# ZencashOfficial/ginger-lib

Measured on AMD Instinct MI355X. Metric: MNT4-753 G1 MSM scalar-muls/sec + 2^n NTT ms at 1/2/4/8 MI355X, higher is better.
Workload: dtype u32 (29-bit limbs of 753-bit Montgomery residues, 64-bit accumulators)

## Files before the change

ginger-lib_amd/__init__.py:

```python
import ctypes
import os

import numpy as np

_PKG_DIR = os.path.dirname(os.path.abspath(__file__))
LIB_PATH = os.path.join(_PKG_DIR, "libginger_hip.so")

GH_OK = 0
FFT_INVERSE = 1
FFT_COSET = 2

CURVES = {"mnt4753_g1": 0, "mnt4753_g2": 1, "mnt6753_g1": 2, "mnt6753_g2": 3}
CURVE_DEG = {"mnt4753_g1": 1, "mnt4753_g2": 2, "mnt6753_g1": 1, "mnt6753_g2": 3}
FIELDS = {"mnt4753_fr": 0, "mnt6753_fr": 1}

ABI_SYMBOLS = [
    "gh_init", "gh_shutdown", "gh_last_error", "gh_device_name",
    "gh_msm", "gh_bases_upload", "gh_bases_upload_wire", "gh_bases_generate_chain", "gh_bases_download", "gh_bases_free", "gh_bases_len", "gh_bases_precompute", "gh_bases_precomputed_window", "gh_bases_precompute_rows", "gh_bases_table_rows",
    "gh_msm_resident", "gh_msm_resident_dev", "gh_msm_resident_dev_batch",
    "gh_msm_cached", "gh_key_cache_config", "gh_key_cache_clear", "gh_key_cache_stats", "gh_bases_content_hash",
    "gh_bases_key_id", "gh_test_hooks",
    "gh_msm_set_window", "gh_msm_set_affine", "gh_msm_set_dedup", "gh_msm_get_window", "gh_msm_last_timing", "gh_msm_batch_timing",
    "gh_domain_supported", "gh_fft", "gh_fft_dev", "gh_vec_mul_dev", "gh_vec_sub_dev", "gh_vec_scale_dev",
    "gh_vec_mul", "gh_vec_scale", "gh_fft_last_kernel_ms", "gh_measure_fpmul_peak", "gh_kernel_resources", "gh_witness_map", "gh_witness_map_dev",
# ... 159 lines not shown

    def download(self, dtype=np.uint64):
        out = np.empty(self.nbytes // np.dtype(dtype).itemsize, dtype=dtype)
        _check(load_library().gh_dev_download(_ptr(out), self.ptr, out.nbytes))
        return out

    def free(self):
        if self.ptr:
            load_library().gh_dev_free(self.ptr)
            self.ptr = ctypes.c_void_p()

    def __enter__(self):
        return self

    def __exit__(self, *exc):
        self.free()


def msm_cached(curve, bases, scalars, infinity=None):
    deg = CURVE_DEG[curve]
    bases = _u64(bases, 24 * deg)
    scalars = _u64(scalars, 12)
    inf = None if infinity is None else np.ascontiguousarray(infinity, dtype=np.uint8)
    out = np.zeros(36 * deg, dtype=np.uint64)
    _check(load_library().gh_msm_cached(CURVES[curve], _ptr(bases), _ptr(inf) if inf is not None else None, bases.size // (24 * deg),
                                        _ptr(scalars), scalars.size // 12, _ptr(out)))
    return out


def key_cache_config(max_bytes=None, table_after=2):
    _check(load_library().gh_key_cache_config((1 << 64) - 1 if max_bytes is None else int(max_bytes), int(table_after)))


def key_cache_clear():
    _check(load_library().gh_key_cache_clear())


def key_cache_stats():
    st = KeyCacheStats()
    _check(load_library().gh_key_cache_stats(ctypes.byref(st)))
    return {k: int(getattr(st, k)) for k, _ in KeyCacheStats._fields_}


def bases_content_hash(curve, bases, infinity=None):
    deg = CURVE_DEG[curve]
    bases = _u64(bases, 24 * deg)
    inf = None if infinity is None else np.ascontiguousarray(infinity, dtype=np.uint8)
    hi = ctypes.c_uint64(0)
    lo = load_library().gh_bases_content_hash(CURVES[curve], _ptr(bases), _ptr(inf) if inf is not None else None, bases.size // (24 * deg), ctypes.byref(hi))
    return int(lo), int(hi.value)


def measure_fpmul_peak():
    v = ctypes.c_double(0)
    _check(load_library().gh_measure_fpmul_peak(ctypes.byref(v)))
    return float(v.value)


def kernel_resources(which):
    a, b, c = ctypes.c_uint32(0), ctypes.c_uint32(0), ctypes.c_uint32(0)
    _check(load_library().gh_kernel_resources(which.encode(), ctypes.byref(a), ctypes.byref(b), ctypes.byref(c)))
    return {"scratch_bytes_per_lane": int(a.value), "registers": int(b.value), "lds_bytes": int(c.value)}


def acc_stamps(max_records=1 << 16):
    buf = np.zeros((max_records, 16), dtype=np.uint32)
    n = ctypes.c_uint32(0)
    fn = load_library().gh_acc_stamps_read
    fn.argtypes = [ctypes.POINTER(ctypes.c_uint32), ctypes.c_size_t, ctypes.POINTER(ctypes.c_uint32)]
    _check(fn(buf.ctypes.data_as(ctypes.POINTER(ctypes.c_uint32)), buf.size, ctypes.byref(n)))
    return buf[:int(n.value)]


def bases_key_id(curve, bases, infinity=None):
    deg = CURVE_DEG[curve]
    bases = _u64(bases, 24 * deg)
    inf = None if infinity is None else np.ascontiguousarray(infinity, dtype=np.uint8)
    out = (ctypes.c_uint64 * 4)()
    _check(load_library().gh_bases_key_id(CURVES[curve], _ptr(bases), _ptr(inf) if inf is not None else None, bases.size // (24 * deg), out))
    return tuple(int(x) for x in out)


def set_test_hooks(flags):
    _check(load_library().gh_test_hooks(int(flags)))


class ResidentBases:

    def __init__(self, curve, bases, infinity=None):
        self.curve = curve
        deg = CURVE_DEG[curve]
        bases = _u64(bases, 24 * deg)
        n = bases.size // (24 * deg)
        inf = None
        if infinity is not None:
            inf = np.ascontiguousarray(infinity, dtype=np.uint8)
            assert inf.size == n
        self.handle = ctypes.c_void_p()
        _check(load_library().gh_bases_upload(CURVES[curve], _ptr(bases), _ptr(inf) if inf is not None else None, n,
                                               ctypes.byref(self.handle)))
        self.n = n

    @classmethod
    def from_wire(cls, curve, data):
        buf = np.frombuffer(bytes(data), dtype=np.uint8)
        rec = 192 * CURVE_DEG[curve] + 1
        if buf.size % rec:
            raise ValueError("wire data is not a multiple of %d bytes" % rec)
        self = cls.__new__(cls)
        self.curve = curve
        self.n = buf.size // rec
        self.handle = ctypes.c_void_p()
        _check(load_library().gh_bases_upload_wire(CURVES[curve], _ptr(buf), self.n, ctypes.byref(self.handle)))
        return self

    @classmethod
    def chain(cls, curve, p0_xy, step_xy, n):
        self = cls.__new__(cls)
        self.curve, self.n = curve, int(n)
        self.handle = ctypes.c_void_p()
        p0, st = _u64(p0_xy), _u64(step_xy)
        _check(load_library().gh_bases_generate_chain(CURVES[curve], _ptr(p0), _ptr(st), self.n, ctypes.byref(self.handle)))
        return self

    def download(self, first, count):
        out = np.zeros((int(count), 24 * CURVE_DEG[self.curve]), dtype=np.uint64)
        _check(load_library().gh_bases_download(self.handle, int(first), int(count), _ptr(out)))
        return out

    def precompute(self, window_bits=0, max_rows=0):
        _check(load_library().gh_bases_precompute_rows(self.handle, int(window_bits), int(max_rows)))
        return load_library().gh_bases_precomputed_window(self.handle)

    def table_rows(self):
        return load_library().gh_bases_table_rows(self.handle)

    def msm(self, scalars):
        scalars = _u64(scalars, 12)
        out = np.zeros(36 * CURVE_DEG[self.curve], dtype=np.uint64)
        _check(load_library().gh_msm_resident(self.handle, _ptr(scalars), scalars.size // 12, _ptr(out)))
        return out

    def msm_dev(self, d_scalars, n_scalars):
        out = np.zeros(36 * CURVE_DEG[self.curve], dtype=np.uint64)
        _check(load_library().gh_msm_resident_dev(self.handle, d_scalars.ptr, n_scalars, _ptr(out)))
        return out

    def free(self):
        if self.handle:
            load_library().gh_bases_free(self.handle)
            self.handle = ctypes.c_void_p()


def msm_batch_dev(jobs):
    if not jobs:
        return []
    k = len(jobs)
    deg = CURVE_DEG[jobs[0][0].curve]
    handles = (ctypes.c_void_p * k)(*[j[0].handle for j in jobs])
    scal = (ctypes.c_void_p * k)(*[j[1].ptr for j in jobs])
    ns = (ctypes.c_size_t * k)(*[int(j[2]) for j in jobs])
    out = np.zeros(k * 36 * deg, dtype=np.uint64)
    _check(load_library().gh_msm_resident_dev_batch(handles, scal, ns, k, _ptr(out)))
    return [out[i * 36 * deg:(i + 1) * 36 * deg].copy() for i in range(k)]


class VariableBaseMSM:

    @staticmethod
    def multi_scalar_mul(curve, bases, scalars, infinity=None):
        deg = CURVE_DEG[curve]
        bases = _u64(bases, 24 * deg)
        scalars = _u64(scalars, 12)
        n_b, n_s = bases.size // (24 * deg), scalars.size // 12
        inf = None
        if infinity is not None:
            inf = np.ascontiguousarray(infinity, dtype=np.uint8)
            assert inf.size == n_b
        out = np.zeros(36 * deg, dtype=np.uint64)
        _check(load_library().gh_msm(CURVES[curve], _ptr(bases), _ptr(inf) if inf is not None else None, n_b,
                                      _ptr(scalars), n_s, _ptr(out)))
        return out


class FixedBaseMSM:

    @staticmethod
    def get_mul_window_size(num_scalars):
        return load_library().gh_fixed_base_window(int(num_scalars))

    def __init__(self, curve, g_xyz, scalar_size=753, window=None, num_scalars=0):
        self.curve = curve
        self.window = int(window) if window else self.get_mul_window_size(num_scalars)
        g = _u64(g_xyz)
        assert g.size == 36 * CURVE_DEG[curve]
        self.handle = ctypes.c_void_p()
        _check(load_library().gh_fixed_base_table(CURVES[curve], _ptr(g), int(scalar_size), self.window, ctypes.byref(self.handle)))

    def multi_scalar_mul(self, scalars):
        s = _u64(scalars, 12)
        n = s.size // 12
        out = np.zeros((n, 36 * CURVE_DEG[self.curve]), dtype=np.uint64)
        _check(load_library().gh_fixed_base_msm(self.handle, _ptr(s), n, _ptr(out)))
        return out

    def multi_scalar_mul_affine(self, scalars, canonical=False):
        s = _u64(scalars, 12)
        n = s.size // 12
        xy = np.zeros((n, 24 * CURVE_DEG[self.curve]), dtype=np.uint64)
        inf = np.zeros(n, dtype=np.uint8)
        _check(load_library().gh_fixed_base_msm_affine(self.handle, _ptr(s), n, _ptr(xy), _ptr(inf), 1 if canonical else 0))
        return xy, inf

    def free(self):
        if self.handle:
            load_library().gh_fixed_base_free(self.handle)
            self.handle = ctypes.c_void_p()


def msm_set_window(c):
    _check(load_library().gh_msm_set_window(int(c)))


def msm_set_affine(mode):
    _check(load_library().gh_msm_set_affine(int(mode)))


def msm_set_dedup(on):
    _check(load_library().gh_msm_set_dedup(1 if on else 0))


def dev_trim():
    _check(load_library().gh_dev_trim())


def msm_last_timing():
    t = MsmTiming()
    _check(load_library().gh_msm_last_timing(ctypes.byref(t)))
    return {k: getattr(t, k) for k, _ in MsmTiming._fields_}


def msm_batch_timing(index):
    t = MsmTiming()
    _check(load_library().gh_msm_batch_timing(int(index), ctypes.byref(t)))
    return {k: getattr(t, k) for k, _ in MsmTiming._fields_}


def proj_add(curve, acc, p):
    acc = _u64(acc).copy()
    p = _u64(p)
    _check(load_library().gh_proj_add(CURVES[curve], _ptr(acc), _ptr(p)))
    return acc


def proj_mul(curve, xyz, scalar12):
    xyz = _u64(xyz)
    k = _u64(scalar12, 12)
    out = np.zeros_like(xyz)
    _check(load_library().gh_proj_mul(CURVES[curve], _ptr(xyz), _ptr(k), _ptr(out)))
    return out


def proj_neg(curve, xyz):
    out = _u64(xyz).copy()
    _check(load_library().gh_proj_neg(CURVES[curve], _ptr(out)))
    return out


_FIELD_ONE = {}


def field_one(curve):
    if curve not in _FIELD_ONE:
        deg = CURVE_DEG[curve]
        z = proj_mul(curve, np.zeros(36 * deg, dtype=np.uint64), np.zeros(12, dtype=np.uint64))
        _FIELD_ONE[curve] = z[12 * deg:24 * deg].copy()
    return _FIELD_ONE[curve]


def proj_to_affine(curve, xyz):
    deg = CURVE_DEG[curve]
    xyz = _u64(xyz)
    out = np.zeros(24 * deg, dtype=np.uint64)
    inf = np.zeros(1, dtype=np.uint8)
    _check(load_library().gh_proj_to_affine(CURVES[curve], _ptr(xyz), _ptr(out), _ptr(inf)))
    return out, bool(inf[0])


class EvaluationDomain:

    def __init__(self, field, num_coeffs):
        lg = ctypes.c_uint32()
        ok = load_library().gh_domain_supported(FIELDS[field], int(num_coeffs), ctypes.byref(lg))
        if not ok:
            raise GingerHipError("domain of 2^%d exceeds the 2-adicity of %s" % (lg.value, field))
        self.field = field
        self.log_size_of_group = lg.value
        self.size = 1 << lg.value

    @classmethod
    def new(cls, field, num_coeffs):
        try:
            return cls(field, num_coeffs)
        except GingerHipError:
            return None

    def _run(self, a, flags):
        a = _u64(a, 12)
        out = np.empty(self.size * 12, dtype=np.uint64)
        _check(load_library().gh_fft(FIELDS[self.field], _ptr(a), a.size // 12, _ptr(out), self.log_size_of_group, flags))
        return out

    def fft(self, coeffs):
        return self._run(coeffs, 0)

    def ifft(self, evals):
        return self._run(evals, FFT_INVERSE)
# ... 64 lines not shown
```

ginger-lib_amd/csrc/ginger_hip.hip:

```cpp
#include <atomic>
#include <condition_variable>
#include <exception>
#include <new>
#include <random>
#include <thread>
#include <stdlib.h>
#include <string.h>
#include <vector>
#include "runtime.h"
#include "scan_kernels.h"
#include "asm_kernels.h"

namespace gh_rt {

Ctx g;
std::string g_err;
static std::mutex g_mu;
std::mutex& api_mutex() { return g_mu; }
static char g_devname[256] = "";
static int g_device_req = -1;

int ensure_init() {
    if (g.ready) return GH_OK;
    int count = 0;
    hipError_t e = hipGetDeviceCount(&count);
    if (e != hipSuccess || count == 0) {
        g_err = "no HIP device visible (this library has no CPU fallback)";
        return GH_E_NO_DEVICE;
    }
    int dev = 0;
    const char* lr = getenv("LOCAL_RANK");
    if (g_device_req >= 0) dev = g_device_req;
    else if (lr) dev = atoi(lr) % count;
    g.device = dev;
    HIPCHK(hipSetDevice(dev));
    hipDeviceProp_t prop;
    HIPCHK(hipGetDeviceProperties(&prop, dev));
    g.num_cus = prop.multiProcessorCount > 0 ? prop.multiProcessorCount : 256;
    snprintf(g_devname, sizeof g_devname, "%s, %d CUs, %s", prop.name, prop.multiProcessorCount, prop.gcnArchName);
    if (strncmp(prop.gcnArchName, "gfx950", 6) != 0) {
        g_err = std::string("device is not gfx950: ") + prop.gcnArchName;
        return GH_E_NO_DEVICE;
    }
    HIPCHK(hipStreamCreate(&g.stream));
    {
        int least = 0, greatest = 0;
        HIPCHK(hipDeviceGetStreamPriorityRange(&least, &greatest));
        auto prio = [&](const char* env, int dflt) {
            const char* v = getenv(env);
            if (!v) return dflt;
            if (!strcmp(v, "low")) return least;
            if (!strcmp(v, "high")) return greatest;
            return (least + greatest) / 2;
        };
        HIPCHK(hipStreamCreateWithPriority(&g.stream_acc, hipStreamDefault, prio("GH_PRIO_ACC", least)));
        HIPCHK(hipStreamCreateWithPriority(&g.stream_red, hipStreamDefault, prio("GH_PRIO_RED", greatest)));
        HIPCHK(hipStreamCreateWithPriority(&g.stream_acc2, hipStreamDefault, prio("GH_PRIO_ACC", least)));
        if (msm_knobs().acc_alt) HIPCHK(hipStreamCreateWithPriority(&g.stream_acc_alt, hipStreamDefault, prio("GH_PRIO_ACC", least)));
    }
    for (auto& ev : g.tev) HIPCHK(hipEventCreateWithFlags(&ev, hipEventDisableTiming));
    for (auto& ev : g.ev) HIPCHK(hipEventCreate(&ev));
    for (auto& sl : g.pev) for (auto& ev : sl) HIPCHK(hipEventCreate(&ev));
    g.ready = true;
    return GH_OK;
}

int api_exception() noexcept {
    int rc = GH_E_HIP;
    const char* what = "unknown C++ exception";
    char buf[384];
    try {
        throw;
    } catch (const std::bad_alloc&) {
        rc = GH_E_NOMEM;
        what = "out of host memory (std::bad_alloc)";
    } catch (const std::exception& e) {
        snprintf(buf, sizeof buf, "C++ exception inside the library: %s", e.what());
        what = buf;
    } catch (...) {
    }
    try {
        std::lock_guard<std::mutex> lk(g_mu);
        g_err = what;
    } catch (...) {
    }
    return rc;
}

int scratch_guard(const void* kernel, size_t threads) {
    static std::map<const void*, size_t> frames;
    size_t& reserved = g.scratch_reserved;
    auto it = frames.find(kernel);
    if (it == frames.end()) {
        hipFuncAttributes a;
        memset(&a, 0, sizeof a);
        size_t f = 0;
        if (hipFuncGetAttributes(&a, kernel) == hipSuccess) f = a.localSizeBytes;
        else (void)hipGetLastError();
        it = frames.emplace(kernel, f).first;
    }
    const size_t frame = it->second;
    if (frame < 1024) return GH_OK;
    const size_t resident = (size_t)g.num_cus * 32 * 64;
    const size_t lanes = threads < resident ? (threads + 63) / 64 * 64 : resident;
    const size_t need = frame * lanes;
    if (need <= reserved) return GH_OK;
    size_t free_b = 0, total_b = 0;
    if (hipMemGetInfo(&free_b, &total_b) != hipSuccess) { (void)hipGetLastError(); return GH_OK; }
    const size_t margin = (size_t)256 << 20;
    if (free_b < need - reserved + margin) {
        char b[256];
        snprintf(b, sizeof b, "not enough device memory for the kernel's stack frames: %zu B per lane x %zu lanes = %zu MB of scratch, %zu MB free",
                 frame, lanes, need >> 20, free_b >> 20);
        g_err = b;
        return GH_E_NOMEM;
    }
    reserved = need;
    return GH_OK;
}

int pool_get(const char* name, size_t bytes, void** out) {
    DevBuf& b = g.pool[name];
    if (b.cap < bytes) {
        if (b.p) {
            HIPCHK(hipDeviceSynchronize());
            HIPCHK(hipFree(b.p));
            b.p = nullptr;
            b.cap = 0;
        }
        size_t cap = bytes + bytes / 8 + 256;
        HIPCHK(hipMalloc(&b.p, cap));
        b.cap = cap;
    }
    *out = b.p;
    return GH_OK;
}

size_t pool_cap(const char* name) {
    auto it = g.pool.find(name);
    return it == g.pool.end() ? 0 : it->second.cap;
}
void pool_release(const char* prefix) {
    const size_t len = strlen(prefix);
    for (auto it = g.pool.begin(); it != g.pool.end();) {
        if (it->first.compare(0, len, prefix) == 0) {
            if (it->second.p) (void)hipFree(it->second.p);
            it = g.pool.erase(it);
        } else {
            ++it;
        }
    }
}
void pool_trim(const char* prefix, size_t keep_bytes) {
    const size_t len = strlen(prefix);
    bool synced = false;
    for (auto it = g.pool.begin(); it != g.pool.end();) {
        if (it->first.compare(0, len, prefix) != 0 || it->second.cap <= keep_bytes) {
            ++it;
            continue;
        }
        if (!synced) (void)hipStreamSynchronize(g.stream);
        synced = true;
        (void)hipFree(it->second.p);
        it = g.pool.erase(it);
    }
}

int device_scan(const uint32_t* in, uint32_t* out, size_t n, const char* tmpname, hipStream_t stream) {
    using namespace gh;
    if (!stream) stream = g.stream;
    size_t per_block = (size_t)SCAN_BLOCK * SCAN_ITEMS;
    size_t nblocks = (n + per_block - 1) / per_block;
    uint32_t* sums;
    int rc = pool_get(tmpname, (nblocks + 1) * 4, (void**)&sums);
    if (rc) return rc;
    GH_LAUNCH(scan_partials_kernel, dim3((unsigned)nblocks), dim3(SCAN_BLOCK), 0, stream, in, sums, n);
    GH_LAUNCH(scan_block_sums_kernel, dim3(1), dim3(1024), 0, stream, sums, nblocks);
    GH_LAUNCH(scan_final_kernel, dim3((unsigned)nblocks), dim3(SCAN_BLOCK), 0, stream, in, sums, out, n);
    HIPCHK(hipGetLastError());
    return GH_OK;
}

const MsmOps* ops_of(gh_curve_t curve) {
    switch (curve) {
        case GH_MNT4753_G1: return msm_ops_mnt4753_g1();
        case GH_MNT4753_G2: return msm_ops_mnt4753_g2();
        case GH_MNT6753_G1: return msm_ops_mnt6753_g1();
        case GH_MNT6753_G2: return msm_ops_mnt6753_g2();
        default: g_err = "unknown curve id"; return nullptr;
    }
}

static int to_device(void* d_dst, const void* h_src, size_t bytes) {
    HIPCHK(hipMemcpyAsync(d_dst, h_src, bytes, hipMemcpyHostToDevice, g.stream));
    return GH_OK;
}
static int to_host_sync(void* h_dst, const void* d_src, size_t bytes) {
    HIPCHK(hipMemcpyAsync(h_dst, d_src, bytes, hipMemcpyDeviceToHost, g.stream));
    HIPCHK(hipStreamSynchronize(g.stream));
    return GH_OK;
}

}

using namespace gh_rt;

extern "C" {

int gh_init(const int* devices, int n_devices) try {
    std::lock_guard<std::mutex> lk(g_mu);
    if (g.ready) return GH_OK;
    if (devices && n_devices > 0) {
        int count = 0;
        if (hipGetDeviceCount(&count) != hipSuccess || count == 0) { g_err = "no HIP device visible"; return GH_E_NO_DEVICE; }
        if (devices[0] < 0 || devices[0] >= count) { g_err = "device index out of range"; return GH_E_BAD_ARG; }
        g_device_req = devices[0];
    }
    return ensure_init();
} catch (...) { return gh_rt::api_exception(); }

int gh_shutdown(void) try {
    std::lock_guard<std::mutex> lk(g_mu);
    dist_teardown_locked();
    if (!g.ready) return GH_OK;
    (void)sync_msm_streams();
    pool_release("");
    for (auto& f : g.at_shutdown) f();
    g.at_shutdown.clear();
    for (int f = 0; f < 2; f++) {
        for (auto& kv : g.domains[f]) kv.second.release();
        g.domains[f].clear();
    }
    for (auto& ev : g.ev) hipEventDestroy(ev);
    for (auto& sl : g.pev) for (auto& ev : sl) hipEventDestroy(ev);
    for (auto& ev : g.tev) hipEventDestroy(ev);
    hipStreamDestroy(g.stream_acc);
    hipStreamDestroy(g.stream_acc2);
    if (g.stream_acc_alt) hipStreamDestroy(g.stream_acc_alt);
    g.stream_acc_alt = nullptr;
    hipStreamDestroy(g.stream_red);
    hipStreamDestroy(g.stream);
    g.scratch_reserved = 0;
    g.ready = false;
    return GH_OK;
} catch (...) { return gh_rt::api_exception(); }

const char* gh_last_error(void) try {
    static thread_local std::string tl;
    std::lock_guard<std::mutex> lk(g_mu);
    tl = g_err;
    return tl.c_str();
} catch (...) { (void)gh_rt::api_exception(); return "C++ exception inside the library"; }
const char* gh_device_name(void) try {
    std::lock_guard<std::mutex> lk(g_mu);
    if (ensure_init()) return "";
    return g_devname;
} catch (...) { (void)gh_rt::api_exception(); return "C++ exception inside the library"; }

int gh_msm(gh_curve_t curve, const uint64_t* bases, const uint8_t* infinity, size_t n_bases, const uint64_t* scalars,
           size_t n_scalars, uint64_t* out_xyz) try {
    std::lock_guard<std::mutex> lk(g_mu);
    if (!out_xyz || (n_bases && !bases) || (n_scalars && !scalars)) { g_err = "null argument"; return GH_E_BAD_ARG; }
    const MsmOps* ops = ops_of(curve);
    if (!ops) return GH_E_BAD_ARG;
    int rc = ensure_init();
    if (rc) return rc;
    return ops->host(bases, infinity, n_bases, scalars, n_scalars, out_xyz);
} catch (...) { return gh_rt::api_exception(); }

int gh_bases_upload(gh_curve_t curve, const uint64_t* bases, const uint8_t* infinity, size_t n_bases, gh_bases_t* out_handle) try {
    std::lock_guard<std::mutex> lk(g_mu);
    if (!out_handle || (n_bases && !bases)) { g_err = "null argument"; return GH_E_BAD_ARG; }
    const MsmOps* ops = ops_of(curve);
    if (!ops) return GH_E_BAD_ARG;
    int rc = ensure_init();
    if (rc) return rc;
    BasesBase* h = nullptr;
    rc = ops->upload(bases, infinity, n_bases, 0, &h);
    if (rc) return rc;
    *out_handle = reinterpret_cast<gh_bases_t>(h);
    return GH_OK;
} catch (...) { return gh_rt::api_exception(); }

int gh_bases_upload_wire(gh_curve_t curve, const uint8_t* bytes, size_t n_points, gh_bases_t* out_handle) try {
    std::lock_guard<std::mutex> lk(g_mu);
    if (!out_handle || (n_points && !bytes)) { g_err = "null argument"; return GH_E_BAD_ARG; }
    const MsmOps* ops = ops_of(curve);
    if (!ops) return GH_E_BAD_ARG;
    int rc = ensure_init();
    if (rc) return rc;
    const int deg = curve_deg(curve);
    static const uint64_t p4[12] = GH_P4_P_64, p6[12] = GH_P6_P_64;
    const uint64_t* mod = (curve == GH_MNT4753_G1 || curve == GH_MNT4753_G2) ? p4 : p6;
    const size_t rec = (size_t)192 * deg + 1, words = (size_t)24 * deg;
    std::vector<uint64_t> xy(n_points * words);
    std::vector<uint8_t> inf(n_points);
    for (size_t i = 0; i < n_points; i++) {
        const uint8_t* r = bytes + i * rec;
        memcpy(&xy[i * words], r, 192 * (size_t)deg);
        if (r[rec - 1] > 1) { g_err = "wire format: infinity flag is not 0 / 1 (bool::read fails)"; return GH_E_BAD_ARG; }
        inf[i] = r[rec - 1];
        for (size_t e = 0; e < 2 * (size_t)deg; e++) {
            const uint64_t* v = &xy[i * words + 12 * e];
            bool lt = false;
            for (int k = 11; k >= 0; k--) { if (v[k] != mod[k]) { lt = v[k] < mod[k]; break; } }
            if (!lt) { g_err = "wire format: coordinate is not a canonical field element"; return GH_E_BAD_ARG; }
        }
    }
    BasesBase* h = nullptr;
    rc = ops->upload(xy.data(), inf.data(), n_points, 1, &h);
    if (rc) return rc;
    *out_handle = reinterpret_cast<gh_bases_t>(h);
    return GH_OK;
} catch (...) { return gh_rt::api_exception(); }

int gh_bases_free(gh_bases_t handle) try {
    std::lock_guard<std::mutex> lk(g_mu);
    BasesBase* h = bases_of(handle);
    if (!h) { g_err = "bad bases handle"; return GH_E_BAD_HANDLE; }
    delete h;
    return GH_OK;
} catch (...) { return gh_rt::api_exception(); }

int gh_bases_precompute_rows(gh_bases_t handle, int window_bits, int max_rows) try {
    std::lock_guard<std::mutex> lk(g_mu);
    BasesBase* h = bases_of(handle);
    if (!h) { g_err = "bad bases handle"; return GH_E_BAD_HANDLE; }
    if (window_bits < 0 || window_bits == 1 || window_bits > 24) { g_err = "window must be 0 (auto) or in [2, 24]"; return GH_E_BAD_ARG; }
    if (max_rows < 0) { g_err = "max_rows must be 0 (no cap) or positive"; return GH_E_BAD_ARG; }
    const MsmOps* ops = ops_of(h->curve);
    if (!ops) return GH_E_BAD_ARG;
    int rc = ensure_init();
    if (rc) return rc;
    return ops->precompute(h, window_bits, max_rows);
} catch (...) { return gh_rt::api_exception(); }
int gh_bases_precompute(gh_bases_t handle, int window_bits) { return gh_bases_precompute_rows(handle, window_bits, 0); }
int gh_bases_table_rows(gh_bases_t handle) try {
    const BasesBase* h = bases_of(handle);
    return h && h->d_table ? h->pre_W : 0;
} catch (...) { return gh_rt::api_exception(); }

int gh_bases_precomputed_window(gh_bases_t handle) try {
    const BasesBase* h = bases_of(handle);
    return h && h->d_table ? h->pre_c : 0;
} catch (...) { return gh_rt::api_exception(); }

size_t gh_bases_len(gh_bases_t handle) try {
    const BasesBase* h = bases_of(handle);
    return h ? h->n : 0;
} catch (...) { (void)gh_rt::api_exception(); return 0; }

int gh_msm_resident_dev(gh_bases_t handle, const void* d_scalars, size_t n_scalars, uint64_t* out_xyz) try {
    std::lock_guard<std::mutex> lk(g_mu);
    BasesBase* h = bases_of(handle);
    if (!h) { g_err = "bad bases handle"; return GH_E_BAD_HANDLE; }
    if (!out_xyz || (n_scalars && !d_scalars)) { g_err = "null argument"; return GH_E_BAD_ARG; }
    const MsmOps* ops = ops_of(h->curve);
    if (!ops) return GH_E_BAD_ARG;
    int rc = ensure_init();
    if (rc) return rc;
    return ops->run(h, d_scalars, n_scalars, out_xyz);
} catch (...) { return gh_rt::api_exception(); }

int gh_msm_resident_dev_batch(const gh_bases_t* handles, const void* const* d_scalars, const size_t* n_scalars, int count,
                              uint64_t* out_xyz) try {
    std::lock_guard<std::mutex> lk(g_mu);
    if (count < 0 || (count > 0 && (!handles || !d_scalars || !n_scalars || !out_xyz))) { g_err = "null argument"; return GH_E_BAD_ARG; }
    if (count == 0) return GH_OK;
    std::vector<BasesBase*> hs((size_t)count);
    for (int i = 0; i < count; i++) {
        BasesBase* h = bases_of(handles[i]);
        if (!h) { g_err = "bad bases handle"; return GH_E_BAD_HANDLE; }
        hs[(size_t)i] = h;
        if (h->curve != hs[0]->curve) { g_err = "a batch must stay on one curve"; return GH_E_BAD_ARG; }
        if (n_scalars[i] && !d_scalars[i]) { g_err = "null argument"; return GH_E_BAD_ARG; }
    }
    const MsmOps* ops = ops_of(hs[0]->curve);
    if (!ops) return GH_E_BAD_ARG;
    int rc = ensure_init();
    if (rc) return rc;
    rc = ops->batch(hs.data(), d_scalars, n_scalars, count, out_xyz);
    if (rc) {
        (void)sync_msm_streams();
    }
    return rc;
} catch (...) { return gh_rt::api_exception(); }

int gh_msm_resident(gh_bases_t handle, const uint64_t* scalars, size_t n_scalars, uint64_t* out_xyz) try {
    std::lock_guard<std::mutex> lk(g_mu);
    BasesBase* h = bases_of(handle);
    if (!h) { g_err = "bad bases handle"; return GH_E_BAD_HANDLE; }
    if (!out_xyz || (n_scalars && !scalars)) { g_err = "null argument"; return GH_E_BAD_ARG; }
    const MsmOps* ops = ops_of(h->curve);
    if (!ops) return GH_E_BAD_ARG;
    int rc = ensure_init();
    if (rc) return rc;
    const size_t n = h->n < n_scalars ? h->n : n_scalars;
    void* d_s = nullptr;
    if (n > 0) {
        rc = pool_get("scalars", n * 96, &d_s);
        if (rc) return rc;
        HIPCHK(hipMemcpyAsync(d_s, scalars, n * 96, hipMemcpyHostToDevice, g.stream));
    }
    return ops->run(h, d_s, n, out_xyz);
} catch (...) { return gh_rt::api_exception(); }

namespace {
struct KeyHash { uint64_t a, b, c, d; };
inline uint64_t rotl64(uint64_t x, int r) { return (x << r) | (x >> (64 - r)); }
inline void hash_words(const uint64_t* w, size_t n, uint64_t& h1, uint64_t& h2, uint64_t& h3, uint64_t& h4) {
    for (size_t i = 0; i < n; i++) {
        const uint64_t x = w[i];
        h1 = rotl64((h1 ^ x) * 0x9E3779B97F4A7C15ull, 29) + 0xD6E8FEB86659FD93ull;
        h2 = (rotl64(h2, 31) + x) * 0xC2B2AE3D27D4EB4Full ^ (h2 >> 33);
        h3 = rotl64(h3 + x * 0xFF51AFD7ED558CCDull, 27) * 0x94D049BB133111EBull ^ x;
        h4 = (h4 ^ rotl64(x, 17)) * 0xD1342543DE82EF95ull + (h4 >> 29);
    }
}
struct HashSeeds { uint64_t s[4]; };
const HashSeeds& hash_seeds() {
    static const HashSeeds hs = [] {
        HashSeeds v;
        try {
            std::random_device rd;
            for (auto& x : v.s) x = ((uint64_t)rd() << 32) ^ (uint64_t)rd() ^ 0x5851F42D4C957F2Dull;
        } catch (...) {
            uint64_t t = (uint64_t)std::chrono::steady_clock::now().time_since_epoch().count() ^ (uint64_t)(uintptr_t)&v;
            for (auto& x : v.s) { t = t * 6364136223846793005ull + 1442695040888963407ull; x = t; }
        }
        return v;
    }();
    return hs;
}
int g_test_hooks = 0;

class HashPool {
public:
    static HashPool& get() { static HashPool* p = new HashPool(); return *p; }
    void run(size_t n, const std::function<void(size_t)>& fn) {
        if (n == 0) return;
        std::unique_lock<std::mutex> one(submit_);
        if (n == 1 || workers_ == 0) { for (size_t c = 0; c < n; c++) fn(c); return; }
        {
            std::lock_guard<std::mutex> lk(mu_);
            fn_ = &fn; n_ = n; next_.store(0); pending_ = workers_; gen_++;
        }
        cv_.notify_all();
        work();
        std::unique_lock<std::mutex> lk(mu_);
        done_.wait(lk, [&] { return pending_ == 0; });
        fn_ = nullptr;
    }
private:
    HashPool() {
        unsigned nt = std::thread::hardware_concurrency();
        nt = nt == 0 ? 1 : (nt > 32 ? 32 : nt);
        for (unsigned t = 1; t < nt; t++) {
            try {
                std::thread([this] { loop(); }).detach();
                workers_++;
            } catch (...) {
                break;
            }
        }
    }
    void work() {
        for (;;) {
            const size_t c = next_.fetch_add(1);
            if (c >= n_) return;
            (*fn_)(c);
        }
    }
    void loop() {
        uint64_t seen = 0;
        for (;;) {
            {
                std::unique_lock<std::mutex> lk(mu_);
                cv_.wait(lk, [&] { return gen_ != seen; });
                seen = gen_;
            }
            work();
            std::lock_guard<std::mutex> lk(mu_);
            if (--pending_ == 0) done_.notify_all();
        }
    }
    std::mutex submit_, mu_;
    std::condition_variable cv_, done_;
    const std::function<void(size_t)>* fn_ = nullptr;
    size_t n_ = 0;
    std::atomic<size_t> next_{0};
    unsigned workers_ = 0, pending_ = 0;
    uint64_t gen_ = 0;
};

KeyHash content_hash(gh_curve_t curve, const uint64_t* bases, const uint8_t* infinity, size_t n) {
    const size_t words = n * (size_t)24 * curve_deg(curve);
    const HashSeeds& sd = hash_seeds();
    const size_t chunk = (size_t)1 << 16;
    const size_t n_chunks = (words + chunk - 1) / chunk;
    std::vector<uint64_t> ch(4 * n_chunks + 4);
    HashPool::get().run(n_chunks, [&](size_t c) {
        uint64_t h1 = sd.s[0] + c, h2 = sd.s[1] ^ c, h3 = sd.s[2] - c, h4 = sd.s[3] ^ (c * 0x9E3779B97F4A7C15ull);
        const size_t lo = c * chunk, len = words - lo < chunk ? words - lo : chunk;
        hash_words(bases + lo, len, h1, h2, h3, h4);
        ch[4 * c] = h1; ch[4 * c + 1] = h2; ch[4 * c + 2] = h3; ch[4 * c + 3] = h4;
    });
    uint64_t h1 = sd.s[1] ^ (uint64_t)curve, h2 = sd.s[0] + n, h3 = sd.s[3] + (uint64_t)curve * 0x100000001B3ull, h4 = sd.s[2] ^ n;
    hash_words(ch.data(), 4 * n_chunks, h1, h2, h3, h4);
    if (infinity) {
        uint64_t any = 0;
        std::vector<uint64_t> fw((n + 63) / 64 + 1, 0);
        for (size_t i = 0; i < n; i++) if (infinity[i]) { fw[i >> 6] |= 1ull << (i & 63); any = 1; }
        if (any) hash_words(fw.data(), fw.size(), h1, h2, h3, h4);
    }
    if (g_test_hooks & 1) { h1 = 0x1111111111111111ull; h2 = 0x2222222222222222ull; }
    return KeyHash{h1, h2, h3, h4};
}
struct CachedKey {
    gh_curve_t curve;
    size_t n;
    KeyHash h;
    BasesBase* key;
    uint64_t stamp;
    uint32_t sightings;
    size_t bytes;
};
struct KeyCache {
    std::vector<CachedKey> e;
    uint64_t clock = 0;
    size_t max_bytes = 0;
    bool budget_set = false;
    int table_after = 2;
    gh_key_cache_stats_t st{};
    bool registered = false;
    void* d_scal = nullptr;
    size_t scal_cap = 0;
};
KeyCache kc;
size_t key_bytes(const BasesBase* h) {
    const size_t pt = (size_t)208 * curve_deg(h->curve);
    return h->n * pt + (h->d_inf ? h->n : 0) + (h->d_table ? (size_t)h->pre_W * h->n * pt : 0) + (size_t)4 * (h->n_dup_groups + 1 + h->n_dup_members);
}
void cache_drop_all() {
    for (auto& k : kc.e) delete k.key;
    kc.e.clear();
    kc.st.entries = 0; kc.st.bytes = 0;
}
void cache_fit(const BasesBase* keep) {
    for (;;) {
        size_t total = 0;
        for (auto& k : kc.e) total += k.bytes;
        kc.st.bytes = total; kc.st.entries = kc.e.size();
        if (total <= kc.max_bytes) return;
        size_t victim = kc.e.size();
        for (size_t i = 0; i < kc.e.size(); i++)
            if (kc.e[i].key != keep && (victim == kc.e.size() || kc.e[i].stamp < kc.e[victim].stamp)) victim = i;
        if (victim == kc.e.size()) return;
        (void)sync_msm_streams();
        delete kc.e[victim].key;
        kc.e.erase(kc.e.begin() + (long)victim);
        kc.st.evictions++;
    }
}
}

uint64_t gh_bases_content_hash(gh_curve_t curve, const uint64_t* bases, const uint8_t* infinity, size_t n_bases, uint64_t* hi) try {
    if (n_bases && !bases) return 0;
    const KeyHash h = content_hash(curve, bases, infinity, n_bases);
    if (hi) *hi = h.b;
    return h.a;
} catch (...) { (void)gh_rt::api_exception(); return 0; }

int gh_bases_key_id(gh_curve_t curve, const uint64_t* bases, const uint8_t* infinity, size_t n_bases, uint64_t* out4) try {
    if (!out4 || (n_bases && !bases)) { std::lock_guard<std::mutex> lk(g_mu); g_err = "null argument"; return GH_E_BAD_ARG; }
    const KeyHash h = content_hash(curve, bases, infinity, n_bases);
    out4[0] = h.a; out4[1] = h.b; out4[2] = h.c; out4[3] = h.d;
    return GH_OK;
} catch (...) { return gh_rt::api_exception(); }

int gh_test_hooks(int flags) try {
    std::lock_guard<std::mutex> lk(g_mu);
    g_test_hooks = flags;
    return GH_OK;
} catch (...) { return gh_rt::api_exception(); }

int gh_key_cache_config(size_t max_bytes, int table_after) try {
    std::lock_guard<std::mutex> lk(g_mu);
    if (table_after < 0) { g_err = "table_after must be >= 0"; return GH_E_BAD_ARG; }
    kc.budget_set = max_bytes != GH_KEY_CACHE_AUTO;
    kc.max_bytes = kc.budget_set ? max_bytes : 0;
    kc.table_after = table_after;
    if (g.ready && kc.budget_set) cache_fit(nullptr);
    return GH_OK;
} catch (...) { return gh_rt::api_exception(); }
int gh_key_cache_clear(void) try {
    std::lock_guard<std::mutex> lk(g_mu);
    if (g.ready) (void)sync_msm_streams();
    cache_drop_all();
    return GH_OK;
} catch (...) { return gh_rt::api_exception(); }
int gh_key_cache_stats(gh_key_cache_stats_t* out) try {
    std::lock_guard<std::mutex> lk(g_mu);
    if (!out) { g_err = "null argument"; return GH_E_BAD_ARG; }
    *out = kc.st;
    return GH_OK;
} catch (...) { return gh_rt::api_exception(); }

int gh_msm_cached(gh_curve_t curve, const uint64_t* bases, const uint8_t* infinity, size_t n_bases, const uint64_t* scalars,
                  size_t n_scalars, uint64_t* out_xyz) try {
    if (!out_xyz || (n_bases && !bases) || (n_scalars && !scalars)) {
        std::lock_guard<std::mutex> lk(g_mu);
        g_err = "null argument";
        return GH_E_BAD_ARG;
    }
    const size_t n = n_bases < n_scalars ? n_bases : n_scalars;
    std::lock_guard<std::mutex> lk(g_mu);
    const MsmOps* ops = ops_of(curve);
    if (!ops) return GH_E_BAD_ARG;
    int rc = ensure_init();
    if (rc) return rc;
    void* d_s = nullptr;
    hipError_t up_err = hipSuccess;
    std::thread uploader;
    struct Joiner { std::thread& t; ~Joiner() { if (t.joinable()) t.join(); } } joiner{uploader};
    if (n > 0) {
        if (kc.scal_cap < n * 96) {
            if (kc.d_scal) { HIPCHK(hipFree(kc.d_scal)); kc.d_scal = nullptr; kc.scal_cap = 0; }
            HIPCHK(hipMalloc(&kc.d_scal, n * 96 + 256));
            kc.scal_cap = n * 96;
        }
        d_s = kc.d_scal;
        const int dev = g.device;
        hipStream_t st = g.stream;
        try {
            uploader = std::thread([=, &up_err] {
                hipError_t e = hipSetDevice(dev);
                if (e == hipSuccess) e = hipMemcpyAsync(d_s, scalars, n * 96, hipMemcpyHostToDevice, st);
                up_err = e;
            });
        } catch (...) {
            HIPCHK(hipMemcpyAsync(d_s, scalars, n * 96, hipMemcpyHostToDevice, st));
        }
    }
    const KeyHash hh = content_hash(curve, bases, infinity, n);
    if (!kc.registered) {
        kc.registered = true;
        g.at_shutdown.push_back([] {
            cache_drop_all();
            if (kc.d_scal) (void)hipFree(kc.d_scal);
            kc.d_scal = nullptr; kc.scal_cap = 0;
            kc.registered = false;
        });
    }
    if (!kc.budget_set) {
        size_t free_b = 0, total_b = 0;
        HIPCHK(hipMemGetInfo(&free_b, &total_b));
        kc.max_bytes = free_b / 2;
        kc.budget_set = true;
    }
    CachedKey* hit = nullptr;
    for (auto& k : kc.e) {
        if (k.curve != curve || k.n != n || k.h.a != hh.a || k.h.b != hh.b) continue;
        if (k.h.c != hh.c || k.h.d != hh.d) { kc.st.collisions++; continue; }
        hit = &k;
        break;
    }
    if (!hit) {
        kc.st.misses++;
        BasesBase* h = nullptr;
        rc = ops->upload(bases, infinity, n, 0, &h);
        if (rc == GH_E_NOMEM && !kc.e.empty()) {
            (void)hipGetLastError();
            (void)sync_msm_streams();
            cache_drop_all();
            rc = ops->upload(bases, infinity, n, 0, &h);
        }
        if (rc) return rc;
        kc.e.push_back(CachedKey{curve, n, hh, h, 0, 0, key_bytes(h)});
        hit = &kc.e.back();
    } else {
        kc.st.hits++;
    }
    hit->stamp = ++kc.clock;
    hit->sightings++;
    BasesBase* key = hit->key;
    if (kc.table_after > 0 && hit->sightings == (uint32_t)kc.table_after && !key->d_table && n >= 4096) {
        const size_t row_bytes = key_bytes(key);
        size_t max_rows = row_bytes ? (kc.max_bytes / 4) / row_bytes : 0;
        if (max_rows > 4096) max_rows = 4096;
        const int prc = max_rows >= 2 ? ops->precompute(key, 0, (int)max_rows)
                                      : GH_E_NOMEM;
        if (prc == GH_OK) kc.st.tables_built++;
        else (void)hipGetLastError();
        hit->bytes = key_bytes(key);
    }
    cache_fit(key);
    if (uploader.joinable()) uploader.join();
    HIPCHK(up_err);
    return ops->run(key, d_s, n, out_xyz);
} catch (...) { return gh_rt::api_exception(); }

int gh_msm_set_window(int c) try {
    std::lock_guard<std::mutex> lk(g_mu);
    if (c < 0 || c > 24 || c == 1) { g_err = "window must be 0 (auto) or in [2, 24]"; return GH_E_BAD_ARG; }
    g.window_override = c;
    return GH_OK;
} catch (...) { return gh_rt::api_exception(); }
int gh_msm_set_affine(int on) try {
    std::lock_guard<std::mutex> lk(g_mu);
    if (on < 0 || on > 2) { g_err = "affine mode must be 0 (off), 1 (on) or 2 (automatic)"; return GH_E_BAD_ARG; }
    g.affine_mode = on;
    return GH_OK;
} catch (...) { return gh_rt::api_exception(); }
int gh_msm_set_dedup(int on) try {
    std::lock_guard<std::mutex> lk(g_mu);
    g.dedup_mode = on ? 1 : 0;
    return GH_OK;
} catch (...) { return gh_rt::api_exception(); }
int gh_msm_get_window(gh_curve_t curve, size_t n) try {
    std::lock_guard<std::mutex> lk(g_mu);
    return auto_window(n, curve_deg(curve));
} catch (...) { return gh_rt::api_exception(); }
int gh_msm_batch_timing(int index, gh_msm_timing_t* out) try {
    std::lock_guard<std::mutex> lk(g_mu);
    if (index < 0 || (size_t)index >= g.batch_tm.size()) { g_err = "no such MSM in the last batch"; return GH_E_BAD_ARG; }
    if (out) *out = g.batch_tm[(size_t)index];
    return GH_OK;
} catch (...) { return gh_rt::api_exception(); }
int gh_msm_last_timing(gh_msm_timing_t* out) try {
    std::lock_guard<std::mutex> lk(g_mu);
    if (out) *out = g.last_msm;
    return GH_OK;
} catch (...) { return gh_rt::api_exception(); }

int gh_domain_supported(gh_field_t field, size_t num_coeffs, uint32_t* log_n) try {
    size_t size = 1;
    uint32_t lg = 0;
    while (size < num_coeffs) { size <<= 1; lg++; }
    if (log_n) *log_n = lg;
    int two_adicity = field == GH_MNT4753_FR ? GH_P6_TWO_ADICITY : GH_P4_TWO_ADICITY;
    return (int)lg < two_adicity ? 1 : 0;
} catch (...) { return gh_rt::api_exception(); }

int gh_fft_dev(gh_field_t field, void* d_data, uint32_t log_n, uint32_t flags) try {
    std::lock_guard<std::mutex> lk(g_mu);
    if (!d_data) { g_err = "null argument"; return GH_E_BAD_ARG; }
    int rc = ensure_init();
    if (rc) return rc;
    return fft_run(field, d_data, log_n, flags);
} catch (...) { return gh_rt::api_exception(); }

int gh_fft(gh_field_t field, const uint64_t* in, size_t n_in, uint64_t* out, uint32_t log_n, uint32_t flags) try {
    if (!out || (n_in && !in)) { std::lock_guard<std::mutex> lk(g_mu); g_err = "null argument"; return GH_E_BAD_ARG; }
    if (log_n >= 31) { std::lock_guard<std::mutex> lk(g_mu); g_err = "domain too large"; return GH_E_UNSUPPORTED; }
    const size_t N = (size_t)1 << log_n;
    std::lock_guard<std::mutex> lk(g_mu);
    int rc = ensure_init();
    if (rc) return rc;
    int two_adicity = field == GH_MNT4753_FR ? GH_P6_TWO_ADICITY : GH_P4_TWO_ADICITY;
    if ((int)log_n >= two_adicity) { g_err = "domain exceeds the field's 2-adicity"; return GH_E_UNSUPPORTED; }
    void* d = nullptr;
    rc = pool_get("fft_io", N * 96, &d);
    if (rc) return rc;
    size_t ncopy = n_in < N ? n_in : N;
    if (ncopy) HIPCHK(hipMemcpyAsync(d, in, ncopy * 96, hipMemcpyHostToDevice, g.stream));
    if (ncopy < N) HIPCHK(hipMemsetAsync((char*)d + ncopy * 96, 0, (N - ncopy) * 96, g.stream));
    rc = fft_run(field, d, log_n, flags);
    if (rc) return rc;
    HIPCHK(hipMemcpyAsync(out, d, N * 96, hipMemcpyDeviceToHost, g.stream));
    HIPCHK(hipStreamSynchronize(g.stream));
    return GH_OK;
} catch (...) { return gh_rt::api_exception(); }

int gh_witness_map_dev(gh_field_t field, void* d_a, void* d_b, void* d_c, uint32_t log_n, const uint64_t* d1,
                       const uint64_t* d2, const uint64_t* d3, void* d_h) try {
    std::lock_guard<std::mutex> lk(g_mu);
    if (!d_a || !d_b || !d_c || !d_h || !d1 || !d2 || !d3) { g_err = "null argument"; return GH_E_BAD_ARG; }
    int rc = ensure_init();
    if (rc) return rc;
    return witness_map(field, d_a, d_b, d_c, log_n, d1, d2, d3, d_h);
} catch (...) { return gh_rt::api_exception(); }

int gh_witness_map(gh_field_t field, const uint64_t* a, const uint64_t* b, const uint64_t* c, uint32_t log_n,
                   const uint64_t* d1, const uint64_t* d2, const uint64_t* d3, uint64_t* h) try {
    std::lock_guard<std::mutex> lk(g_mu);
    if (!a || !b || !c || !h || !d1 || !d2 || !d3) { g_err = "null argument"; return GH_E_BAD_ARG; }
    if (log_n >= 31) { g_err = "domain too large"; return GH_E_UNSUPPORTED; }
    const size_t bytes = ((size_t)1 << log_n) * 96;
    int rc = ensure_init();
    if (rc) return rc;
    DevMem da, db, dc, dh;
    if ((rc = da.alloc(bytes)) || (rc = db.alloc(bytes)) || (rc = dc.alloc(bytes)) || (rc = dh.alloc(bytes + 96))) return rc;
    if ((rc = to_device(da.get(), a, bytes)) || (rc = to_device(db.get(), b, bytes)) || (rc = to_device(dc.get(), c, bytes))) return rc;
    if ((rc = witness_map(field, da.get(), db.get(), dc.get(), log_n, d1, d2, d3, dh.get()))) return rc;
    return to_host_sync(h, dh.get(), bytes + 96);
} catch (...) { return gh_rt::api_exception(); }

int gh_sap_witness_map_dev(gh_field_t field, void* d_a, void* d_c, uint32_t log_n, const uint64_t* d1, const uint64_t* d2, void* d_h) try {
    std::lock_guard<std::mutex> lk(g_mu);
    if (!d_a || !d_c || !d_h || !d1 || !d2) { g_err = "null argument"; return GH_E_BAD_ARG; }
    int rc = ensure_init();
    if (rc) return rc;
    return sap_witness_map(field, d_a, d_c, log_n, d1, d2, d_h);
} catch (...) { return gh_rt::api_exception(); }

int gh_sap_witness_map(gh_field_t field, const uint64_t* a, const uint64_t* c, uint32_t log_n, const uint64_t* d1, const uint64_t* d2, uint64_t* h) try {
    std::lock_guard<std::mutex> lk(g_mu);
    if (!a || !c || !h || !d1 || !d2) { g_err = "null argument"; return GH_E_BAD_ARG; }
    if (log_n >= 31) { g_err = "domain too large"; return GH_E_UNSUPPORTED; }
    const size_t bytes = ((size_t)1 << log_n) * 96;
    int rc = ensure_init();
    if (rc) return rc;
    DevMem da, dc, dh;
    if ((rc = da.alloc(bytes)) || (rc = dc.alloc(bytes)) || (rc = dh.alloc(bytes + 96))) return rc;
    if ((rc = to_device(da.get(), a, bytes)) || (rc = to_device(dc.get(), c, bytes))) return rc;
    if ((rc = sap_witness_map(field, da.get(), dc.get(), log_n, d1, d2, dh.get()))) return rc;
    return to_host_sync(h, dh.get(), bytes + 96);
} catch (...) { return gh_rt::api_exception(); }

int gh_batch_inverse_dev(gh_field_t field, void* d_a, size_t n) try {
    std::lock_guard<std::mutex> lk(g_mu);
    if (n && !d_a) { g_err = "null argument"; return GH_E_BAD_ARG; }
    int rc = ensure_init();
    if (rc) return rc;
    return batch_inverse(field, d_a, n);
} catch (...) { return gh_rt::api_exception(); }

int gh_batch_inverse(gh_field_t field, uint64_t* a, size_t n) try {
    if (n == 0) return GH_OK;
    std::lock_guard<std::mutex> lk(g_mu);
    if (!a) { g_err = "null argument"; return GH_E_BAD_ARG; }
    int rc = ensure_init();
    if (rc) return rc;
    DevMem da;
    if ((rc = da.alloc(n * 96)) || (rc = to_device(da.get(), a, n * 96)) || (rc = batch_inverse(field, da.get(), n))) return rc;
    return to_host_sync(a, da.get(), n * 96);
} catch (...) { return gh_rt::api_exception(); }

int gh_lagrange_coefficients_dev(gh_field_t field, uint32_t log_n, const uint64_t* tau12, void* d_out) try {
    std::lock_guard<std::mutex> lk(g_mu);
    if (!tau12 || !d_out) { g_err = "null argument"; return GH_E_BAD_ARG; }
    if (log_n >= 31) { g_err = "domain too large"; return GH_E_UNSUPPORTED; }
    int rc = ensure_init();
    if (rc) return rc;
    return lagrange_coefficients(field, log_n, tau12, d_out);
} catch (...) { return gh_rt::api_exception(); }

int gh_lagrange_coefficients(gh_field_t field, uint32_t log_n, const uint64_t* tau12, uint64_t* out) try {
    std::lock_guard<std::mutex> lk(g_mu);
    if (!tau12 || !out) { g_err = "null argument"; return GH_E_BAD_ARG; }
    if (log_n >= 31) { g_err = "domain too large"; return GH_E_UNSUPPORTED; }
    const size_t bytes = ((size_t)1 << log_n) * 96;
// ... 152 lines not shown
```

ginger-lib_amd/csrc/msm_impl.h:

```cpp
#pragma once
#include <stdlib.h>
#include <string.h>
#include <chrono>
#include <memory>
#include <type_traits>
#include <vector>
#include "runtime.h"
#include "msm_kernels.h"
#include "asm_kernels.h"
#include "msm_plan.h"
#include "msm_fold.h"
#include "msm_key.h"

namespace gh_rt {
using namespace gh;

template <class C> struct GenConst;
template <> struct GenConst<Mnt4G1> { static void get(uint64_t* xy) { static const uint64_t x[12] = GH_MNT4753_G1_GX0_M_64, y[12] = GH_MNT4753_G1_GY0_M_64; memcpy(xy, x, 96); memcpy(xy + 12, y, 96); } };
template <> struct GenConst<Mnt6G1> { static void get(uint64_t* xy) { static const uint64_t x[12] = GH_MNT6753_G1_GX0_M_64, y[12] = GH_MNT6753_G1_GY0_M_64; memcpy(xy, x, 96); memcpy(xy + 12, y, 96); } };
template <> struct GenConst<Mnt4G2> { static void get(uint64_t* xy) {
    static const uint64_t x0[12] = GH_MNT4753_G2_GX0_M_64, x1[12] = GH_MNT4753_G2_GX1_M_64, y0[12] = GH_MNT4753_G2_GY0_M_64, y1[12] = GH_MNT4753_G2_GY1_M_64;
    memcpy(xy, x0, 96); memcpy(xy + 12, x1, 96); memcpy(xy + 24, y0, 96); memcpy(xy + 36, y1, 96); } };
template <> struct GenConst<Mnt6G2> { static void get(uint64_t* xy) {
    static const uint64_t x0[12] = GH_MNT6753_G2_GX0_M_64, x1[12] = GH_MNT6753_G2_GX1_M_64, x2[12] = GH_MNT6753_G2_GX2_M_64;
    static const uint64_t y0[12] = GH_MNT6753_G2_GY0_M_64, y1[12] = GH_MNT6753_G2_GY1_M_64, y2[12] = GH_MNT6753_G2_GY2_M_64;
    memcpy(xy, x0, 96); memcpy(xy + 12, x1, 96); memcpy(xy + 24, x2, 96); memcpy(xy + 36, y0, 96); memcpy(xy + 48, y1, 96); memcpy(xy + 60, y2, 96); } };

template <class C> MsmModulus scalar_modulus() {
    static const uint32_t r4[24] = GH_P6_P_32, r6[24] = GH_P4_P_32;
    const bool mnt4 = CurveId<C>::id == GH_MNT4753_G1 || CurveId<C>::id == GH_MNT4753_G2;
    MsmModulus m;
    memcpy(m.w, mnt4 ? r4 : r6, sizeof m.w);
    return m;
}

template <class C> int make_salts(Aff<C>* out) {
    typedef typename C::F F;
    uint64_t xy[72];
    GenConst<C>::get(xy);
    const uint32_t* w = reinterpret_cast<const uint32_t*>(xy);
    out[0].x = F::from_abi(w);
    out[0].y = F::from_abi(w + 24 * F::DEG);
    Proj<C> g2 = proj_dbl<C>(Proj<C>{out[0].x, out[0].y, F::one()});
    typename F::T zi = host_inv<F>(g2.z);
    out[1].x = F::mul(g2.x, zi);
    out[1].y = F::mul(g2.y, zi);
    return GH_OK;
}

template <class C> int device_salts(Aff<C>** out) {
    static Aff<C>* d_salts = nullptr;
    if (!d_salts) {
        Aff<C> hs[2];
        if (int src = make_salts<C>(hs)) return src;
        HIPCHK(hipMalloc((void**)&d_salts, sizeof(hs)));
        HIPCHK(hipMemcpy(d_salts, hs, sizeof(hs), hipMemcpyHostToDevice));
        g.at_shutdown.push_back([] { if (d_salts) hipFree(d_salts); d_salts = nullptr; });
    }
    *out = d_salts;
    return GH_OK;
}

template <class C> struct SplitFS {
    typedef typename std::conditional<C::F::DEG == 1, F1S<typename C::PF>,
            typename std::conditional<C::F::DEG == 2, F2S<P4, 13>, F3S<P6, 11>>::type>::type type;
};

template <class C> struct BucketSumArgs {
    const void* points = nullptr;
    const uint32_t *sorted = nullptr, *starts = nullptr, *counts = nullptr, *order = nullptr;
    uint32_t total = 0;
    const Aff<C>* salts = nullptr;
    Proj<C>* out = nullptr;
    const uint32_t* chunk_start = nullptr;
    uint32_t n_heavy = 0, n_chunks = 0, heavy_chunk = 0;
    Proj<C>* partials = nullptr;
    uint32_t bucket0 = 0, in_base = 0;
};
template <class C, bool AFFIN>
int launch_bucket_sums(const BucketSumArgs<C>& a, const std::string& task_pool, hipStream_t st) {
    const size_t tasks = (size_t)a.n_chunks + (a.total - a.n_heavy);
    if constexpr (C::F::DEG == 1) {
        if (!AFFIN && gh_asm::enabled()) {
            gh_asm::AccTask* tk = nullptr;
            if (int rc = pool_get(task_pool.c_str(), tasks * sizeof(gh_asm::AccTask) + 16, (void**)&tk)) return rc;
            uint32_t* const counter = (uint32_t*)(tk + tasks);
            GH_LAUNCH((msm_acc_tasks_kernel<C>), dim3((unsigned)((tasks + 255) / 256)), dim3(256), 0, st, a.starts, a.counts, a.order,
                      a.total, a.out, a.chunk_start, a.n_heavy, a.n_chunks, a.heavy_chunk, a.partials, (AccTaskRec*)tk, counter);
            return gh_asm::acc_g1_launch(std::is_same<typename C::PF, P6>::value ? 6 : 4, a.points, a.sorted, tk, a.salts, (uint32_t)tasks,
                                         counter, st);
        }
        GH_LAUNCH((msm_accumulate_xyzz_kernel<C, AFFIN>), dim3((unsigned)((tasks + 255) / 256)), dim3(256), 0, st,
                  (const Aff<C>*)a.points, a.sorted, a.starts, a.counts, a.order, a.total, a.salts, a.out, a.chunk_start, a.n_heavy,
                  a.n_chunks, a.heavy_chunk, a.partials, a.bucket0, a.in_base);
    } else {
        typedef typename SplitFS<C>::type FS;
        constexpr int LANES = FS::LANES;
        const size_t waves = (tasks + (64 / LANES) - 1) / (64 / LANES);
        GH_LAUNCH((msm_accumulate_split_kernel<C, FS, LANES, AFFIN>), dim3((unsigned)((waves * 64 + 255) / 256)), dim3(256), 0, st,
                  (const Aff<C>*)a.points, a.sorted, a.starts, a.counts, a.order, a.total, a.salts, a.out, a.chunk_start, a.n_heavy,
                  a.n_chunks, a.heavy_chunk, a.partials, a.bucket0, a.in_base);
    }
    return GH_OK;
}

template <class C> struct TreeLists {
    const Aff<C>* rows = nullptr;
    const uint32_t* sorted = nullptr;
    uint32_t* desc = nullptr;
    void *ptsA = nullptr, *ptsB = nullptr, *prefix = nullptr, *stage1 = nullptr, *stage2 = nullptr;
    void* asm_accs = nullptr;
    uint32_t* asm_flag = nullptr;
    size_t accs_half = 0, flag_words = 0;
};

template <class C> struct Piece {
    AffRoundArgs<C> a;
    gh_asm::AffArgs q;
    uint32_t waves_cpp, aw, Bq;
    uint32_t* flag;
    void* accs;
    Piece(const TreePlan& tp, const TreeLists<C>& L, int r, const void* in, void* out, const uint32_t* desc, uint32_t o0,
          uint32_t n_piece, uint32_t in_base, int which) {
        const PieceGeom geo = tp.piece(n_piece, o0);
        auto off = [&](void* base, int chunks) { return (void*)((char*)base + t64_bytes(geo.t0, chunks)); };
        a.rows = L.rows; a.in = in; a.sorted = r == 0 ? L.sorted : nullptr; a.desc = desc; a.n_out = n_piece; a.in_base = in_base;
        a.prefix = off(L.prefix, T64_FP_CHUNKS); a.out = off(out, T64_PT_CHUNKS);
        a.stage1 = off(L.stage1, T64_PT_CHUNKS); a.stage2 = off(L.stage2, T64_PT_CHUNKS);
        a.groups = geo.waves * tp.tpw; a.bmin = tp.bmin;
        a.run_if = nullptr;
        waves_cpp = geo.waves; aw = geo.aw; Bq = geo.Bq;
        flag = L.asm_flag ? L.asm_flag + (size_t)which * L.flag_words : nullptr;
        accs = L.asm_accs ? (void*)((char*)L.asm_accs + (size_t)which * L.accs_half) : nullptr;
        q.in = r == 0 ? (const void*)L.rows : in; q.sorted = L.sorted; q.desc = a.desc; q.prefix = a.prefix;
        q.stage1 = a.stage1; q.stage2 = a.stage2; q.out = a.out; q.accs = accs; q.flag = flag;
        q.n_out = n_piece; q.in_base = in_base; q.B = Bq; q.pad = 0;
    }
};

struct RoundFork {
    hipStream_t st, st2;
    bool open = false;
    RoundFork(hipStream_t st_, hipStream_t st2_) : st(st_), st2(st2_) {}
    RoundFork(const RoundFork&) = delete;
    RoundFork& operator=(const RoundFork&) = delete;
    int fork() {
        HIPCHK(hipEventRecord(g.tev[0], st));
        HIPCHK(hipStreamWaitEvent(st2, g.tev[0], 0));
        open = true;
        return GH_OK;
    }
    int join() {
        open = false;
        HIPCHK(hipEventRecord(g.tev[1], st2));
        HIPCHK(hipStreamWaitEvent(st, g.tev[1], 0));
        return GH_OK;
    }
    ~RoundFork() {
        if (!open) return;
        (void)hipEventRecord(g.tev[1], st2);
        (void)hipStreamWaitEvent(st, g.tev[1], 0);
    }
};

template <class C>
struct MsmJob {
    typedef typename SplitFS<C>::type FS;
    static constexpr int DEG = C::F::DEG;

    BasesBase* h = nullptr;
    const void* d_scalars = nullptr;
    uint64_t* out_xyz = nullptr;
    size_t n = 0;
    int slot = 0;
    bool solo = false;
    bool last = false;
    int es = 0;
    MsmPlan p;
    bool tree = false;
    uint32_t n_heavy = 0, n_chunks = 0;
    int32_t* digits = nullptr;
    uint32_t *counts = nullptr, *starts = nullptr, *cursor = nullptr, *sorted = nullptr, *order = nullptr, *size_hist = nullptr,
             *size_cursor = nullptr, *chunk_start = nullptr, *plan = nullptr;
    Proj<C>*buckets = nullptr, *seg_out = nullptr, *win_out = nullptr, *partials = nullptr, *lane_out = nullptr;
    uint32_t* red_flag = nullptr;
    uint32_t *aff_cnt = nullptr, *aff_st = nullptr;
    bool aff_sticky_pending = false;
    uint32_t* hplan = nullptr;
    Proj<C>* hw = nullptr;
    Aff<C>* salts = nullptr;
    std::chrono::steady_clock::time_point t_begin;
    gh_msm_timing_t tm{};

    static int pinned(int slot, int which, size_t bytes, void** out) {
        static void* p[4][2] = {};
        static size_t cap[4][2] = {};
        static bool registered = false;
        if (!registered) {
            registered = true;
            g.at_shutdown.push_back([] {
                for (auto& sl : p) for (auto& q : sl) { if (q) hipHostFree(q); q = nullptr; }
                for (auto& sl : cap) for (auto& q : sl) q = 0;
                registered = false;
            });
        }
        if (cap[slot][which] < bytes) {
            if (p[slot][which]) HIPCHK(hipHostFree(p[slot][which]));
            p[slot][which] = nullptr; cap[slot][which] = 0;
            HIPCHK(hipHostMalloc(&p[slot][which], bytes + 256, hipHostMallocDefault));
            cap[slot][which] = bytes + 256;
        }
        *out = p[slot][which];
        return GH_OK;
    }

    int prepare(BasesBase* h_, const void* d_scalars_, size_t n_scalars, uint64_t* out, int slot_) {
        h = h_; d_scalars = d_scalars_; out_xyz = out; slot = slot_;
        n = h->n < n_scalars ? h->n : n_scalars;
        t_begin = std::chrono::steady_clock::now();
        if (n == 0) return GH_OK;
        p = plan_msm(n, DEG, h->d_table != nullptr, h->pre_c, h->pre_G, solo, last, g.window_override, g.affine_mode, msm_knobs());
        if (p.status == MSM_PLAN_TOO_LARGE) {
            g_err = "MSM too large for 31-bit list entries";
            return GH_E_UNSUPPORTED;
        }
        tree = p.tree;
        if (int src = device_salts<C>(&salts)) return src;
        int rc;
        if ((rc = slot_buf("digits", slot, p.entries * 4, &digits)) ||
            (rc = slot_buf("counts", slot, p.total * 4, &counts)) ||
            (rc = slot_buf("starts", slot, p.total * 4, &starts)) ||
            (rc = slot_buf("cursor", slot, p.total * 4, &cursor)) ||
            (rc = slot_buf("sorted", slot, p.entries * 4, &sorted)) ||
            (rc = slot_buf("order", slot, p.total * 4, &order)) ||
            (rc = slot_buf("size_hist", slot, MSM_SIZE_BINS * 4, &size_hist)) ||
            (rc = slot_buf("size_cursor", slot, MSM_SIZE_BINS * 4, &size_cursor)) ||
            (rc = slot_buf("chunk_start", slot, (p.max_heavy + 2) * 4, &chunk_start)) ||
            (rc = slot_buf("plan", slot, 64, &plan)) ||
            (rc = slot_buf("buckets", slot, p.total * sizeof(Proj<C>), &buckets)) ||
            (rc = slot_buf("seg_out", slot, (size_t)p.RW * p.segs_per_window * 3 * sizeof(Proj<C>), &seg_out)) ||
            (rc = slot_buf("win_out", slot, (size_t)3 * p.RW * 3 * sizeof(Proj<C>), &win_out)))
            return rc;
        if (p.lane_buf && (rc = slot_buf("lane_out", slot, (size_t)p.RW * p.segs_per_window * 64 * 2 * sizeof(Proj<C>), &lane_out))) return rc;
        if (p.lane_buf && (rc = slot_buf("reduce_flag", slot, (size_t)p.RW * p.segs_per_window * 4 + 64, &red_flag))) return rc;
        if ((rc = pinned(es, 0, 512, (void**)&hplan))) return rc;
        if ((rc = pinned(es, 1, (size_t)9 * p.RW * sizeof(Proj<C>), (void**)&hw))) return rc;
        return GH_OK;
    }

    int merge_equal_bases(hipStream_t st) {
        int rc;
        uint32_t *merged_s = nullptr, *partial = nullptr;
        if ((rc = slot_buf("merged_scalars", slot, n * 96, &merged_s))) return rc;
        HIPCHK(hipMemcpyAsync(merged_s, d_scalars, n * 96, hipMemcpyDeviceToDevice, st));
        if ((rc = slot_buf("merged_partial", slot, (size_t)h->n_dup_chunks * 96 + 96, &partial))) return rc;
        GH_LAUNCH(msm_merge_scalars_kernel, dim3(h->n_dup_chunks), dim3(256), 0, st, (const uint32_t*)d_scalars, merged_s, n,
                  (const uint32_t*)h->d_dup_starts, (const uint32_t*)h->d_dup_members, (const uint32_t*)h->d_dup_chunks, h->n_dup_chunks,
                  partial, scalar_modulus<C>());
        GH_LAUNCH(msm_merge_groups_kernel, dim3((h->n_dup_groups + 63) / 64), dim3(64), 0, st, merged_s, n, (const uint32_t*)h->d_dup_starts,
                  (const uint32_t*)h->d_dup_members, (const uint32_t*)(h->d_dup_chunks + 3 * (size_t)h->n_dup_chunks), h->n_dup_groups,
                  (const uint32_t*)partial, scalar_modulus<C>());
        d_scalars = merged_s;
        return GH_OK;
    }

    int launch_digits(uint32_t* hist, hipStream_t st) {
        GH_LAUNCH(msm_digits_kernel, dim3((unsigned)((n + 255) / 256)), dim3(256), 0, st, (const uint32_t*)d_scalars, (const uint8_t*)h->d_inf,
                  n, p.c, p.W, p.nb, p.top_unsigned, scalar_modulus<C>(), digits, hist, msm_knobs().agg_iters, p.merged ? 1u : 0u, (uint32_t)p.sets);
        return GH_OK;
    }

    int sort_partitioned(const SortPlan& sp, hipStream_t st) {
        int rc;
        MsmPartArgs a;
        a.digits = digits; a.entries = p.entries; a.n = n;
        a.win_stride = p.nb; a.row_stride = p.merged ? (uint32_t)h->n : 0u; a.slot_shift = p.merged ? 1u : 0u;
        a.sets = (uint32_t)p.sets;
        a.bin_shift = sp.bin_shift; a.n_bins = sp.n_bins;
        a.tile = sp.tile; a.n_blocks = sp.n_blocks;
        const size_t cells = (size_t)a.n_bins * a.n_blocks + 1;
        uint32_t *block_hist = nullptr, *block_off = nullptr;
        uint2* part = nullptr;
        if ((rc = slot_buf("part_hist", slot, cells * 4, &block_hist)) ||
            (rc = slot_buf("part_off", slot, cells * 4, &block_off)) ||
            (rc = slot_buf("part_pairs", slot, p.entries * 8, &part))) return rc;
        if ((rc = launch_digits(nullptr, st))) return rc;
        HIPCHK(hipMemsetAsync(block_hist + (cells - 1), 0, 4, st));
        GH_LAUNCH(msm_part_hist_kernel, dim3(a.n_blocks), dim3(MSM_PART_THREADS), 0, st, a, block_hist);
        HIPCHK(hipGetLastError());
        if ((rc = device_scan(block_hist, block_off, cells, slot_name("scan_tmp3", slot).c_str(), st))) return rc;
        GH_LAUNCH(msm_part_scatter_kernel, dim3(a.n_blocks), dim3(MSM_PART_THREADS), 0, st, a, (const uint32_t*)block_off, part);
        GH_LAUNCH(msm_bin_sort_kernel, dim3(a.n_bins), dim3(MSM_BIN_THREADS), (size_t)4 << sp.bin_shift, st, (const uint2*)part,
                  (const uint32_t*)block_off, a.n_blocks, sp.bin_shift, (uint32_t)p.total, counts, starts, sorted);
        HIPCHK(hipGetLastError());
        return GH_OK;
    }

    int launch_sort(hipStream_t st) {
        if (n == 0) return GH_OK;
        int rc;
        const size_t total = p.total;
        HIPCHK(hipEventRecord(g.pev[es][0], st));
        HIPCHK(hipMemsetAsync(size_hist, 0, MSM_SIZE_BINS * 4, st));
        HIPCHK(hipMemsetAsync(plan, 0, 64, st));
        if (h->n_dup_groups && (rc = merge_equal_bases(st))) return rc;
        const SortPlan sp = plan_sort(p.entries, n, total, msm_knobs());
        if (sp.part) {
            if ((rc = sort_partitioned(sp, st))) return rc;
        } else {
            HIPCHK(hipMemsetAsync(counts, 0, total * 4, st));
            if ((rc = launch_digits(counts, st))) return rc;
            HIPCHK(hipGetLastError());
            if ((rc = device_scan(counts, starts, total, "scan_tmp", st))) return rc;
            HIPCHK(hipMemcpyAsync(cursor, starts, total * 4, hipMemcpyDeviceToDevice, st));
        }
        GH_LAUNCH(msm_size_hist_kernel, dim3((unsigned)((total + 255) / 256)), dim3(256), 0, st, counts, total, p.heavy_thr, size_hist, plan + 4);
        if ((rc = device_scan(size_hist, size_cursor, MSM_SIZE_BINS, "scan_tmp2", st))) return rc;
        GH_LAUNCH(msm_size_scatter_kernel, dim3((unsigned)((total + 255) / 256)), dim3(256), 0, st, counts, total, p.heavy_thr, size_cursor, order);
        GH_LAUNCH(msm_heavy_plan_kernel, dim3(1), dim3(1), 0, st, (const uint32_t*)size_hist, (const uint32_t*)counts,
                  (const uint32_t*)order, (const uint32_t*)starts, (uint32_t)total, p.heavy_chunk, chunk_start, plan);
        if (!sp.part)
            GH_LAUNCH(msm_scatter_kernel, dim3((unsigned)((n + 255) / 256), (unsigned)p.W), dim3(256), 0, st,
                      (const int32_t*)digits, n, p.W, p.nb, p.merged ? (uint32_t)h->n : 0u, cursor, sorted, msm_knobs().agg_iters,
                      p.merged ? 1u : 0u, (uint32_t)p.sets);
        HIPCHK(hipGetLastError());
        HIPCHK(hipMemcpyAsync(hplan, plan, 32, hipMemcpyDeviceToHost, st));
        HIPCHK(hipEventRecord(g.pev[es][1], st));
        return GH_OK;
    }

    int launch_accumulate(hipStream_t st) {
        if (n == 0) return GH_OK;
        int rc;
        HIPCHK(hipEventSynchronize(g.pev[es][1]));
        n_heavy = hplan[0]; n_chunks = hplan[1];
        tm.accumulate_madds = hplan[2];
        if (n_heavy > p.max_heavy || n_chunks > p.max_chunks) { g_err = "internal: heavy-bucket plan out of range"; return GH_E_HIP; }
        partials = nullptr;
        if (n_heavy > 0 && (rc = slot_buf("partials", slot, (size_t)n_chunks * sizeof(Proj<C>), &partials))) return rc;
        HIPCHK(hipEventRecord(g.pev[es][2], st));
        if (tree) {
            if ((rc = launch_tree(st))) return rc;
        }
        if (!tree) {
            BucketSumArgs<C> a;
            a.points = p.merged ? h->d_table : h->d_points;
            a.sorted = sorted; a.starts = starts; a.counts = counts; a.order = order; a.total = (uint32_t)p.total;
            a.salts = salts; a.out = buckets;
            a.chunk_start = chunk_start; a.n_heavy = n_heavy; a.n_chunks = n_chunks; a.heavy_chunk = p.heavy_chunk; a.partials = partials;
            if ((rc = launch_bucket_sums<C, false>(a, slot_name("acc_tasks", slot), st))) return rc;
        }
        HIPCHK(hipGetLastError());
        HIPCHK(hipEventRecord(g.pev[es][3], st));
        if (n_heavy > 0) {
            GH_LAUNCH((msm_heavy_combine_kernel<C>), dim3(n_heavy), dim3(64), 64 * sizeof(Proj<C>), st, (const Proj<C>*)partials,
                      (const uint32_t*)order, (const uint32_t*)chunk_start, buckets);
            HIPCHK(hipGetLastError());
        }
        HIPCHK(hipEventRecord(g.pev[es][4], st));
        return GH_OK;
    }

    struct TreeRun {
        TreePlan tp;
        TreeLists<C> L;
        std::vector<uint32_t> bq, tab;
        bool aff_asm = false;
        int asm_kind = 0;
        uint32_t T(uint32_t j, int r) const { return tab[(size_t)j * (tp.R + 1) + r]; }
    };
    const uint32_t* round_starts(const TreeRun& t, int r) const { return r == 0 ? starts : aff_st + (size_t)(r - 1) * t.tp.stride; }
    const uint32_t* round_counts(const TreeRun& t, int r) const { return r == 0 ? counts : aff_cnt + (size_t)(r - 1) * t.tp.stride; }

    int tree_counts(const TreePlan& tp, hipStream_t st) {
        int rc;
        const size_t total = p.total;
        if ((rc = slot_buf("aff_cnt", slot, (size_t)tp.R * tp.stride * 4, &aff_cnt)) ||
            (rc = slot_buf("aff_st", slot, (size_t)tp.R * tp.stride * 4, &aff_st))) return rc;
        GH_LAUNCH(aff_counts_kernel, dim3((unsigned)((total + 255) / 256)), dim3(256), 0, st,
                  (const uint32_t*)counts, (uint32_t)total, tp.R, tp.stride, aff_cnt);
        const std::string scan_nm = slot_name("aff_scan", slot);
        for (int r = 1; r <= tp.R; r++)
            if ((rc = device_scan(aff_cnt + (size_t)(r - 1) * tp.stride, aff_st + (size_t)(r - 1) * tp.stride, total, scan_nm.c_str(), st))) return rc;
        return GH_OK;
    }

    int tree_chunk_tables(TreeRun& t, uint32_t n0, hipStream_t st) {
        int rc;
        const uint32_t K = t.tp.K;
        const int R = t.tp.R;
        uint32_t *d_bq, *d_tab;
        if ((rc = slot_buf("aff_bq", slot, ((size_t)K + 2) * 4, &d_bq)) ||
            (rc = slot_buf("aff_tab", slot, ((size_t)K + 2) * (R + 1) * 4, &d_tab))) return rc;
        GH_LAUNCH(aff_chunks_kernel, dim3((K + 1 + 63) / 64), dim3(64), 0, st, (const uint32_t*)starts, (const uint32_t*)counts,
                  (const uint32_t*)aff_st, (const uint32_t*)aff_cnt, (uint32_t)p.total, R, t.tp.stride, K, d_bq, d_tab);
        HIPCHK(hipGetLastError());
        t.bq.resize((size_t)K + 1);
        t.tab.resize(((size_t)K + 1) * (R + 1));
        HIPCHK(hipMemcpyAsync(t.bq.data(), d_bq, t.bq.size() * 4, hipMemcpyDeviceToHost, st));
        HIPCHK(hipMemcpyAsync(t.tab.data(), d_tab, t.tab.size() * 4, hipMemcpyDeviceToHost, st));
        HIPCHK(hipStreamSynchronize(st));
        if (t.T(K, 0) != n0) { g_err = "internal: affine plan disagrees with the sort stage"; return GH_E_HIP; }
        return GH_OK;
    }

    int tree_lists(TreeRun& t) {
        int rc;
        const int R = t.tp.R;
        uint32_t max_n1 = 0, max_n2 = 0;
        size_t max_desc = 0;
        for (uint32_t j = 0; j < t.tp.K; j++) {
            const uint32_t n1 = t.T(j + 1, 1) - t.T(j, 1), n2 = R >= 2 ? t.T(j + 1, 2) - t.T(j, 2) : 0;
            if (n1 > max_n1) max_n1 = n1;
            if (n2 > max_n2) max_n2 = n2;
            size_t dsum = 0;
            for (int r = 1; r <= R; r++) dsum += t.T(j + 1, r) - t.T(j, r);
            if (dsum > max_desc) max_desc = dsum;
        }
        auto tiles = [&](uint32_t n_el) { return ((size_t)n_el + t.tp.tpw - 1) / t.tp.tpw + 1; };
        TreeLists<C>& L = t.L;
        if ((rc = slot_buf("aff_desc", slot, (max_desc + 64) * 4, &L.desc)) ||
            (rc = slot_buf("aff_ptsA", slot, t64_bytes(tiles(max_n1), T64_PT_CHUNKS), &L.ptsA)) ||
            (rc = slot_buf("aff_ptsB", slot, t64_bytes(tiles(max_n2), T64_PT_CHUNKS), &L.ptsB)) ||
            (rc = slot_buf("aff_prefix", slot, t64_bytes(tiles(max_n1), T64_FP_CHUNKS), &L.prefix)) ||
            (rc = slot_buf("aff_stage1", slot, t64_bytes(tiles(max_n1), T64_PT_CHUNKS), &L.stage1)) ||
            (rc = slot_buf("aff_stage2", slot, t64_bytes(tiles(max_n1), T64_PT_CHUNKS), &L.stage2))) return rc;
        return GH_OK;
    }

    static int issue_fwd(const TreeRun& t, Piece<C>& P, int r, hipStream_t s) {
        HIPCHK(hipMemsetAsync(P.flag, 0, 16, s));
        return gh_asm::aff_launch(t.asm_kind, true, r == 0, P.q, P.aw, s);
    }
    static int issue_rest(const TreeRun& t, Piece<C>& P, int r, hipStream_t s) {
        GH_LAUNCH((aff_inv_kernel<FS>), dim3(P.aw / 4), dim3(256), 0, s, P.accs, P.aw, P.a.n_out, P.Bq, (const uint32_t*)P.flag);
        if (int rc = gh_asm::aff_launch(t.asm_kind, false, r == 0, P.q, P.aw, s)) return rc;
        if (r == 0) GH_LAUNCH((aff_fix_kernel<C, FS, true>), dim3(16), dim3(256), 0, s, P.a, (const uint32_t*)P.flag);
        else GH_LAUNCH((aff_fix_kernel<C, FS, false>), dim3(16), dim3(256), 0, s, P.a, (const uint32_t*)P.flag);
        P.a.run_if = P.flag;
        return GH_OK;
    }
    static int issue_cpp(Piece<C>& P, int r, hipStream_t s) {
        if (r == 0) GH_LAUNCH((aff_round_kernel<C, FS, true>), dim3(P.waves_cpp / 4), dim3(256), 0, s, P.a);
        else GH_LAUNCH((aff_round_kernel<C, FS, false>), dim3(P.waves_cpp / 4), dim3(256), 0, s, P.a);
        return GH_OK;
    }
    static int debug_round(const Piece<C>& P, uint32_t j, int r, uint32_t n_out, hipStream_t st) {
        uint32_t fw[4] = {0, 0, 0, 0};
        HIPCHK(hipStreamSynchronize(st));
        HIPCHK(hipMemcpy(fw, P.flag, 16, hipMemcpyDeviceToHost));
        fprintf(stderr, "[gh aff] chunk %u round %d n_out %u waves %u B %u in_base %u redo %u exceptions %u\n", j, r, n_out, P.aw, P.Bq,
                P.q.in_base, fw[0], fw[1]);
        return GH_OK;
    }

    int issue_round(const TreeRun& t, uint32_t j, int r, uint32_t n_out, const void* in, void* out, uint32_t* desc, hipStream_t st) {
        int rc;
        unsigned dgrid = (n_out + 255) / 256;
        if (dgrid > 16384) dgrid = 16384;
        GH_LAUNCH(aff_desc_kernel, dim3(dgrid), dim3(256), 0, st, round_starts(t, r), round_counts(t, r),
                  (const uint32_t*)(aff_st + (size_t)r * t.tp.stride), (uint32_t)p.total, t.T(j, r + 1), n_out, desc);
        const uint32_t in_base = t.T(j, r);
        const RoundSplit sp = t.tp.split(n_out, t.aff_asm);
        if (!sp.split) {
            Piece<C> P(t.tp, t.L, r, in, out, desc, 0, n_out, in_base, 0);
            if (t.aff_asm) {
                if ((rc = issue_fwd(t, P, r, st)) || (rc = issue_rest(t, P, r, st))) return rc;
                if (msm_knobs().aff_debug && (rc = debug_round(P, j, r, n_out, st))) return rc;
            }
            return issue_cpp(P, r, st);
        }
        Piece<C> A(t.tp, t.L, r, in, out, desc, 0, sp.nA, in_base, 0);
        Piece<C> B(t.tp, t.L, r, in, out, desc + sp.nA, sp.nA, n_out - sp.nA, in_base, 1);
        RoundFork fk(st, g.stream_acc2);
        if ((rc = issue_fwd(t, A, r, st))) return rc;
        if ((rc = fk.fork())) return rc;
        if ((rc = issue_fwd(t, B, r, fk.st2)) ||
            (rc = issue_rest(t, A, r, st)) || (rc = issue_rest(t, B, r, fk.st2)) ||
            (rc = issue_cpp(A, r, st)) || (rc = issue_cpp(B, r, fk.st2))) return rc;
        return fk.join();
    }

    int launch_tree(hipStream_t st) {
        constexpr int LANES = FS::LANES;
        int rc;
        const MsmKnobs& knobs = msm_knobs();
        const uint32_t n0 = hplan[2], maxc = hplan[4];
        TreeRun t{TreePlan(n0, p.total, maxc, DEG, 64 / LANES, (uint32_t)g.num_cus * 4u * (uint32_t)FS::WAVES,
                           (uint32_t)g.num_cus * 4u * 2u , knobs)};
        const int R = t.tp.R;
        if ((rc = tree_counts(t.tp, st))) return rc;
        {
            size_t free_b = 0, total_b = 0;
            HIPCHK(hipMemGetInfo(&free_b, &total_b));
            size_t have = 0;
            const char* names[6] = {"aff_desc", "aff_ptsA", "aff_ptsB", "aff_prefix", "aff_stage1", "aff_stage2"};
            for (const char* nm : names) have += pool_cap(slot_name(nm, slot).c_str());
            if (!t.tp.set_chunks(n0, LANES, free_b, have, knobs)) {
                for (const char* nm : names) pool_release(slot_name(nm, slot).c_str());
                tree = false;
                return GH_OK;
            }
        }
        if ((rc = tree_chunk_tables(t, n0, st))) return rc;
        if ((rc = tree_lists(t))) {
            if (rc != GH_E_NOMEM) return rc;
            (void)hipGetLastError();
            tree = false;
            return GH_OK;
        }
        TreeLists<C>& L = t.L;
        L.rows = (const Aff<C>*)(p.merged ? h->d_table : h->d_points);
        L.sorted = sorted;
        t.aff_asm = (DEG >= 2 ? gh_asm::aff_enabled() : gh_asm::aff_g1_enabled()) && !h->aff_asm_off;
        t.asm_kind = std::is_same<C, Mnt4G2>::value ? 0 : (std::is_same<C, Mnt6G2>::value ? 1 : (std::is_same<C, Mnt6G1>::value ? 3 : 2));
        if (t.aff_asm) {
            L.accs_half = t64_bytes((size_t)t.tp.asm_max_waves + 4, T64_FP_CHUNKS);
            L.flag_words = 16 + (size_t)AFF_FIX_CAP;
            if ((rc = slot_buf("aff_accs", slot, 2 * L.accs_half, &L.asm_accs))) return rc;
            if ((rc = slot_buf("aff_flag", slot, 2 * 4 * L.flag_words, &L.asm_flag))) return rc;
            HIPCHK(hipMemsetAsync(L.asm_flag, 0, 64, st));
            HIPCHK(hipMemsetAsync(L.asm_flag + L.flag_words, 0, 64, st));
        }
        for (uint32_t j = 0; j < t.tp.K; j++) {
            size_t doff = 0;
            const void* in = nullptr;
            for (int r = 0; r < R; r++) {
                const uint32_t n_out = t.T(j + 1, r + 1) - t.T(j, r + 1);
                void* out = (r & 1) ? L.ptsB : L.ptsA;
                if (n_out > 0 && (rc = issue_round(t, j, r, n_out, in, out, L.desc + doff, st))) return rc;
                doff += n_out;
                in = out;
            }
            BucketSumArgs<C> a;
            a.total = t.bq[j + 1] - t.bq[j];
            if (a.total == 0) continue;
            a.points = in; a.starts = round_starts(t, R); a.counts = round_counts(t, R);
            a.salts = salts; a.out = buckets; a.heavy_chunk = p.heavy_chunk;
            a.bucket0 = t.bq[j]; a.in_base = t.T(j, R);
            if ((rc = launch_bucket_sums<C, true>(a, std::string(), st))) return rc;
        }
        HIPCHK(hipGetLastError());
        if (t.aff_asm) {
            HIPCHK(hipMemcpyAsync(&hplan[16], L.asm_flag + 4, 4, hipMemcpyDeviceToHost, st));
            HIPCHK(hipMemcpyAsync(&hplan[17], L.asm_flag + L.flag_words + 4, 4, hipMemcpyDeviceToHost, st));
            aff_sticky_pending = true;
        }
        n_heavy = 0;
        return GH_OK;
    }

    int reduce_level(unsigned grid, const WaveReduceIn<C>& i0, const WaveReduceIn<C>& i1, const WaveReduceIn<C>& i2, uint32_t per_input,
                     uint32_t n_inputs, uint32_t segs, int L, Proj<C>* out, uint32_t* slabs, bool one_wave, hipStream_t st,
                     const uint32_t* run_if = nullptr) {
        if constexpr (DEG >= 2) {
            GH_LAUNCH((msm_wave_reduce_split_kernel<C, FS, FS::LANES, DEG == 2 ? 32 : 16>), dim3(grid), dim3(64), 64 * sizeof(P3), st,
                      i0, i1, i2, per_input, n_inputs, segs, L, (const Aff<C>*)salts, out, slabs);
        } else if (one_wave) {
            GH_LAUNCH((msm_wave_reduce_kernel<C, 1>), dim3(grid), dim3(64), 64 * sizeof(Proj<C>), st,
                      i0, i1, i2, per_input, n_inputs, segs, L, (const Aff<C>*)salts, out, slabs, run_if);
        } else {
            GH_LAUNCH((msm_wave_reduce_kernel<C, 2>), dim3(grid), dim3(64), 64 * sizeof(Proj<C>), st,
                      i0, i1, i2, per_input, n_inputs, segs, L, (const Aff<C>*)salts, out, slabs, run_if);
        }
        return GH_OK;
    }

    int lean_level1(const WaveReduceIn<C>& i0, unsigned nb1, uint32_t segs, uint32_t* slabs, bool one_wave, hipStream_t st) {
        const WaveReduceIn<C> none{nullptr, 0, 0, 0, 0, 0};
        if constexpr (DEG == 1) {
            if (msm_knobs().reduce_waves != 1 && p.L1 >= 2 && red_flag && gh_asm::reduce_enabled()) {
                gh_asm::RedArgs a;
                a.items = i0.base; a.out = lane_out; a.slabs = slabs; a.flag = red_flag;
                a.count = i0.count; a.valid = i0.valid; a.segs = segs; a.L = (uint32_t)p.L1; a.n_programs = nb1; a.pad = 0;
                int rc;
                if ((rc = gh_asm::red_g1_launch(std::is_same<C, Mnt6G1>::value ? 6 : 4, a, (uint32_t)p.RW, st)) ||
                    (rc = reduce_level(nb1, i0, none, none, nb1, 1u, segs, p.L1, lane_out, slabs, false, st, red_flag))) return rc;
                if (msm_knobs().reduce_debug) {
                    std::vector<uint32_t> fw(nb1);
                    HIPCHK(hipStreamSynchronize(st));
                    HIPCHK(hipMemcpy(fw.data(), red_flag, (size_t)nb1 * 4, hipMemcpyDeviceToHost));
                    unsigned redone = 0;
                    for (uint32_t v : fw) redone += v != 0;
                    fprintf(stderr, "reduce: programs %u redone %u\n", nb1, redone);
                }
                return GH_OK;
            }
        }
        return reduce_level(nb1, i0, none, none, nb1, 1u, segs, p.L1, lane_out, slabs, one_wave, st);
    }

    int launch_reduce(hipStream_t st) {
        if (n == 0) return GH_OK;
        int rc;
        const uint32_t RW = (uint32_t)p.RW, segs = p.segs_per_window, all = 0xFFFFFFFFu;
        const unsigned nb1 = RW * segs, nb2 = 3 * RW;
        const WaveReduceIn<C> none{nullptr, 0, 0, 0, 0, 0};
        uint32_t* slabs = nullptr;
        size_t slab_words;
        if constexpr (DEG >= 2) slab_words = WaveSlab<P3>::WORDS; else slab_words = WaveSlab<Proj<C>>::WORDS;
        if ((rc = slot_buf("reduce_slabs", slot, (size_t)(nb1 > nb2 ? nb1 : nb2) * slab_words * 4, &slabs))) return rc;
        const int env_w = msm_knobs().reduce_waves;
        const bool one_wave = env_w ? env_w == 1 : solo;
        if (p.lean) {
            const uint32_t lanes_per_window = segs * 64u;
            const WaveReduceIn<C> i0{buckets, 1, 0, p.Q, 2, (uint32_t)p.total};
            const WaveReduceIn<C> l0{lane_out, 2, 0, lanes_per_window, 0, all}, l1{lane_out, 2, 1, lanes_per_window, 1, all};
            if ((rc = lean_level1(i0, nb1, segs, slabs, one_wave, st)) ||
                (rc = reduce_level(2 * RW, l0, l1, none, RW, 2u, 1u, (int)segs, win_out, slabs, one_wave, st))) return rc;
        } else {
            const WaveReduceIn<C> i0{buckets, 1, 0, p.Q, 0, (uint32_t)p.total};
            const WaveReduceIn<C> r0{seg_out, 3, 0, segs, 0, all}, r1{seg_out, 3, 1, segs, 1, all}, r2{seg_out, 3, 2, segs, 1, all};
            if ((rc = reduce_level(nb1, i0, none, none, nb1, 1u, segs, p.L1, seg_out, slabs, one_wave, st)) ||
                (rc = reduce_level(nb2, r0, r1, r2, RW, 3u, 1u, p.L2, win_out, slabs, one_wave, st))) return rc;
        }
        HIPCHK(hipGetLastError());
        HIPCHK(hipEventRecord(g.pev[es][5], st));
        HIPCHK(hipMemcpyAsync(hw, win_out, (size_t)9 * RW * sizeof(Proj<C>), hipMemcpyDeviceToHost, st));
        HIPCHK(hipEventRecord(g.pev[es][6], st));
        return GH_OK;
    }

    int finish() {
        if (n == 0) {
            proj_to_abi_host<C>(out_xyz, proj_zero<C>());
            g.last_msm = gh_msm_timing_t{};
            g.batch_tm.push_back(g.last_msm);
            return GH_OK;
        }
        HIPCHK(hipEventSynchronize(g.pev[es][6]));
        if (aff_sticky_pending && (hplan[16] != 0 || hplan[17] != 0)) h->aff_asm_off = 1;
        auto t_fold0 = std::chrono::steady_clock::now();
        auto hwv = to_host_curve<C>(hw, (size_t)9 * p.RW);
        if (p.lean) lean_reslot(hwv, p.RW);
        const int u = fold_u(p.sw, p.L1);
        if (p.merged) fold_merged<C>(hwv, p.RW, fold_lq(p.Q), u, p.sw, p.sets, p.c, out_xyz);
        else fold_windows<C>(hwv, p.W, p.c, u, p.sw, p.top_unsigned, out_xyz);
        auto t_end = std::chrono::steady_clock::now();
        HIPCHK(hipEventElapsedTime(&tm.sort_ms, g.pev[es][0], g.pev[es][1]));
        HIPCHK(hipEventElapsedTime(&tm.accumulate_ms, g.pev[es][2], g.pev[es][3]));
        HIPCHK(hipEventElapsedTime(&tm.heavy_ms, g.pev[es][3], g.pev[es][4]));
        HIPCHK(hipEventElapsedTime(&tm.reduce_ms, g.pev[es][4], g.pev[es][5]));
        tm.heavy_buckets = n_heavy;
        tm.fold_ms = std::chrono::duration<float, std::milli>(t_end - t_fold0).count();
        tm.total_ms = std::chrono::duration<float, std::milli>(t_end - t_begin).count();
        tm.window_bits = p.c;
        tm.num_windows = p.W;
        g.last_msm = tm;
        g.batch_tm.push_back(tm);
        return GH_OK;
    }
};

template <class C>
int accumulate_lists(const void* points, const uint32_t* sorted, const uint32_t* starts, const uint32_t* counts,
                     const uint32_t* order, uint32_t total, void* out_proj, hipStream_t st) {
    if (total == 0) return GH_OK;
    Aff<C>* salts = nullptr;
    if (int rc = device_salts<C>(&salts)) return rc;
    BucketSumArgs<C> a;
    a.salts = salts; a.points = points; a.sorted = sorted; a.starts = starts; a.counts = counts; a.order = order; a.total = total;
    a.out = (Proj<C>*)out_proj;
    if (int rc = launch_bucket_sums<C, false>(a, "acc_tasks#lists", st)) return rc;
    HIPCHK(hipGetLastError());
    return GH_OK;
}

template <class C>
int msm_batch(BasesBase* const* hs, const void* const* d_scalars, const size_t* n_scalars, int count, uint64_t* out_xyz) {
    const size_t out_stride = (size_t)36 * C::F::DEG;
    std::vector<MsmJob<C>> jobs((size_t)count);
    int rc;
    auto issue_sort = [&](int k) -> int {
        MsmJob<C>& j = jobs[(size_t)k];
        j.solo = count == 1;
        j.last = k == count - 1;
        j.es = k & 3;
        if ((rc = j.prepare(hs[k], d_scalars[k], n_scalars[k], out_xyz + (size_t)k * out_stride, k & 1))) return rc;
        if (k >= 2) {
            HIPCHK(hipStreamWaitEvent(g.stream, g.pev[(k - 2) & 3][4], 0));
        }
        return j.launch_sort(g.stream);
    };
    g.batch_tm.clear();
    if (count <= 0) return GH_OK;
    if ((rc = issue_sort(0))) return rc;
    for (int k = 0; k < count; k++) {
        MsmJob<C>& j = jobs[(size_t)k];
        const bool alt = C::F::DEG == 1 && g.stream_acc_alt && gh_asm::enabled() && msm_knobs().acc_persist && (k & 1);
        const hipStream_t st_acc = alt ? g.stream_acc_alt : g.stream_acc;
        if (k >= 2 && j.n) HIPCHK(hipStreamWaitEvent(st_acc, g.pev[(k - 2) & 3][6], 0));
        if ((rc = j.launch_accumulate(st_acc))) return rc;
        if (j.n) HIPCHK(hipStreamWaitEvent(g.stream_red, g.pev[k & 3][4], 0));
        if ((rc = j.launch_reduce(g.stream_red))) return rc;
        if (k + 1 < count && (rc = issue_sort(k + 1))) return rc;
        if (k >= 1 && (rc = jobs[(size_t)k - 1].finish())) return rc;
    }
    return jobs[(size_t)count - 1].finish();
}

template <class C>
int msm_run(BasesBase* h, const void* d_scalars, size_t n_scalars, uint64_t* out_xyz) {
    return msm_batch<C>(&h, &d_scalars, &n_scalars, 1, out_xyz);
}

template <class C>
int msm_host(const uint64_t* bases, const uint8_t* infinity, size_t n_bases, const uint64_t* scalars, size_t n_scalars,
             uint64_t* out_xyz) {
    size_t n = n_bases < n_scalars ? n_bases : n_scalars;
    BasesBase* uploaded = nullptr;
    int rc = upload_bases<C>(bases, infinity, n, 0, &uploaded);
    if (rc) return rc;
    const std::unique_ptr<BasesBase> h(uploaded);
    void* d_s = nullptr;
    if (n > 0) {
        if ((rc = pool_get("scalars", n * 96, &d_s))) return rc;
        hipError_t e = hipMemcpyAsync(d_s, scalars, n * 96, hipMemcpyHostToDevice, g.stream);
        if (e != hipSuccess) { g_err = hipGetErrorString(e); return GH_E_HIP; }
    }
    return msm_run<C>(h.get(), d_s, n, out_xyz);
}


#define GH_DEFINE_MSM_OPS(CURVE, NAME)                                                        \
    namespace gh_rt {                                                                          \
    const MsmOps* NAME() {                                                                     \
        static const MsmOps ops = {&upload_bases<CURVE>, &msm_run<CURVE>, &msm_host<CURVE>,    \
                                   &proj_add_host<CURVE>, &to_affine_host<CURVE>,              \
                                   &precompute_bases<CURVE>, &msm_batch<CURVE>,                \
                                   &proj_mul_host<CURVE>, &proj_neg_host<CURVE>, &accumulate_lists<CURVE>};           \
        return &ops;                                                                           \
    }                                                                                          \
    }

}
```

ginger-lib_amd/csrc/runtime.h:

```cpp
#pragma once
#include <hip/hip_runtime.h>
#include <stdint.h>
#include <stdio.h>
#include <stdlib.h>
#include <functional>
#include <map>
#include <mutex>
#include <string>
#include <vector>
#include "../../include/ginger_hip.h"
#include "fp29.h"
#include "msm_plan.h"

struct gh_poseidon;
namespace gh { struct Mnt4G1; struct Mnt4G2; struct Mnt6G1; struct Mnt6G2; }

namespace gh_rt {

template <class T> void dev_free(T*& p) {
    if (p) (void)hipFree(p);
    p = nullptr;
}

struct Domain {
    int log_n = 0;
    gh::Fp* tw = nullptr;
    gh::Fp* coset = nullptr;
    gh::Fp* coset_inv = nullptr;
    gh::Fp size_inv;
    gh::Fp* d_size_inv = nullptr;
    uint32_t* scratch = nullptr;
    uint32_t* scratch2 = nullptr;
    bool scratch2_failed = false;
    void release() { dev_free(tw); dev_free(coset); dev_free(coset_inv); dev_free(d_size_inv); dev_free(scratch); dev_free(scratch2); }
};

struct DevBuf {
    void* p = nullptr;
    size_t cap = 0;
};

struct Ctx {
    bool ready = false;
    int device = 0;
    int num_cus = 256;
    hipStream_t stream = nullptr;
    hipStream_t stream_acc = nullptr;
    hipStream_t stream_red = nullptr;
    hipStream_t stream_acc2 = nullptr;
    hipStream_t stream_acc_alt = nullptr;
    hipEvent_t tev[2] = {nullptr, nullptr};
    hipEvent_t ev[10];
    hipEvent_t pev[4][8];
    std::map<int, Domain> domains[2];
    std::map<std::string, DevBuf> pool;
    int window_override = 0;
    int affine_mode = 2;
    gh_msm_timing_t last_msm{};
    std::vector<gh_msm_timing_t> batch_tm;
    float last_fft_ms = 0;
    int dedup_mode = 1;
    size_t scratch_reserved = 0;
    std::vector<std::function<void()>> at_shutdown;
};

extern Ctx g;
extern std::string g_err;

int ensure_init();
std::mutex& api_mutex();
int pool_get(const char* name, size_t bytes, void** out);
size_t pool_cap(const char* name);
void pool_release(const char* prefix);
void pool_trim(const char* prefix, size_t keep_bytes);
constexpr size_t SLAB_KEEP_BYTES = (size_t)64 << 20;
inline std::string slot_name(const char* name, int slot) { return std::string(name) + "#" + std::to_string(slot); }
template <class T> int slot_buf(const char* name, int slot, size_t bytes, T** out) {
    return pool_get(slot_name(name, slot).c_str(), bytes, (void**)out);
}
inline hipError_t sync_msm_streams() {
    hipError_t e = hipSuccess;
    for (hipStream_t s : {g.stream, g.stream_acc, g.stream_acc2, g.stream_acc_alt, g.stream_red}) {
        if (!s) continue;
        const hipError_t es = hipStreamSynchronize(s);
        if (e == hipSuccess) e = es;
    }
    return e;
}
int device_scan(const uint32_t* in, uint32_t* out, size_t n, const char* tmpname, hipStream_t stream = nullptr);
inline int auto_window(size_t n, int deg) { return auto_window(n, deg, g.window_override); }
void dist_teardown_locked();

int api_exception() noexcept;

int scratch_guard(const void* kernel, size_t threads);
#define GH_LAUNCH(kern, grid, block, shmem, st, ...)                                                              \
    do {                                                                                                          \
        const dim3 g_ = (grid), b_ = (block);                                                                     \
        if (int rc_ = gh_rt::scratch_guard((const void*)(kern), (size_t)g_.x * g_.y * g_.z * b_.x * b_.y * b_.z)) \
            return rc_;                                                                                           \
        hipLaunchKernelGGL(kern, g_, b_, shmem, st, __VA_ARGS__);                                                 \
    } while (0)

#define HIPCHK(call)                                                                         \
    do {                                                                                     \
        hipError_t e_ = (call);                                                              \
        if (e_ != hipSuccess) {                                                              \
            char b_[512];                                                                    \
            snprintf(b_, sizeof b_, "%s failed: %s (%s:%d)", #call, hipGetErrorString(e_), __FILE__, __LINE__); \
            gh_rt::g_err = b_;                                                               \
            return e_ == hipErrorOutOfMemory ? GH_E_NOMEM : GH_E_HIP;                        \
        }                                                                                    \
    } while (0)

class DevMem {
public:
    DevMem() = default;
    DevMem(const DevMem&) = delete;
    DevMem& operator=(const DevMem&) = delete;
    DevMem(DevMem&& o) noexcept : p_(o.release()) {}
    DevMem& operator=(DevMem&& o) noexcept { if (this != &o) { reset(); p_ = o.release(); } return *this; }
    ~DevMem() { reset(); }
    int alloc(size_t bytes) {
        reset();
        HIPCHK(hipMalloc(&p_, bytes));
        return GH_OK;
    }
    void* get() const { return p_; }
    template <class T> T* as() const { return static_cast<T*>(p_); }
    void* release() { void* p = p_; p_ = nullptr; return p; }
    void reset() { dev_free(p_); }
private:
    void* p_ = nullptr;
};

inline int curve_deg(gh_curve_t c) { return c == GH_MNT4753_G2 ? 2 : (c == GH_MNT6753_G2 ? 3 : 1); }
template <class C> struct CurveId;
template <> struct CurveId<gh::Mnt4G1> { static constexpr gh_curve_t id = GH_MNT4753_G1; };
template <> struct CurveId<gh::Mnt4G2> { static constexpr gh_curve_t id = GH_MNT4753_G2; };
template <> struct CurveId<gh::Mnt6G1> { static constexpr gh_curve_t id = GH_MNT6753_G1; };
template <> struct CurveId<gh::Mnt6G2> { static constexpr gh_curve_t id = GH_MNT6753_G2; };
inline int unknown_curve() { g_err = "unknown curve id"; return GH_E_BAD_ARG; }
#define GH_G1_DISPATCH(curve, fn, ...) ((curve) == GH_MNT6753_G1 ? fn<gh::Mnt6G1>(__VA_ARGS__) : fn<gh::Mnt4G1>(__VA_ARGS__))
#define GH_CURVE_DISPATCH(curve, fn, ...)                          \
    ((curve) == GH_MNT4753_G1   ? fn<gh::Mnt4G1>(__VA_ARGS__)       \
     : (curve) == GH_MNT4753_G2 ? fn<gh::Mnt4G2>(__VA_ARGS__)       \
     : (curve) == GH_MNT6753_G1 ? fn<gh::Mnt6G1>(__VA_ARGS__)       \
     : (curve) == GH_MNT6753_G2 ? fn<gh::Mnt6G2>(__VA_ARGS__)       \
                                : gh_rt::unknown_curve())

struct BasesBase {
    gh_curve_t curve;
    size_t n = 0;
    void* d_points = nullptr;
    uint8_t* d_inf = nullptr;
    void* d_table = nullptr;
    int pre_c = 0, pre_W = 0;
    int pre_G = 1;
    uint32_t* d_dup_starts = nullptr;
    uint32_t* d_dup_members = nullptr;
    uint32_t* d_dup_chunks = nullptr;
    uint32_t n_dup_groups = 0, n_dup_members = 0, n_dup_chunks = 0;
    uint8_t aff_asm_off = 0;
    static constexpr uint32_t MAGIC = 0x6768424au;
    uint32_t magic = MAGIC;
    BasesBase() = default;
    BasesBase(const BasesBase&) = delete;
    BasesBase& operator=(const BasesBase&) = delete;
    ~BasesBase() {
        dev_free(d_points); dev_free(d_inf); dev_free(d_table);
        dev_free(d_dup_starts); dev_free(d_dup_members); dev_free(d_dup_chunks);
        magic = 0;
    }
};
inline BasesBase* bases_of(gh_bases_t handle) {
    BasesBase* h = reinterpret_cast<BasesBase*>(handle);
    return h && h->magic == BasesBase::MAGIC ? h : nullptr;
}
struct MsmOps {
    int (*upload)(const uint64_t* bases, const uint8_t* infinity, size_t n, int canonical, BasesBase** out);
    int (*run)(BasesBase* h, const void* d_scalars, size_t n_scalars, uint64_t* out_xyz);
    int (*host)(const uint64_t* bases, const uint8_t* infinity, size_t n_bases, const uint64_t* scalars,
                size_t n_scalars, uint64_t* out_xyz);
    int (*proj_add)(uint64_t* acc_xyz, const uint64_t* p_xyz);
    int (*to_affine)(const uint64_t* xyz, uint64_t* out_xy, uint8_t* is_infinity);
    int (*precompute)(BasesBase* h, int window_bits, int max_rows);
    int (*batch)(BasesBase* const* hs, const void* const* d_scalars, const size_t* n_scalars, int count, uint64_t* out_xyz);
    int (*proj_mul)(const uint64_t* p_xyz, const uint64_t* scalar12, uint64_t* out_xyz);
    int (*proj_neg)(uint64_t* xyz);
    int (*acc_lists)(const void* points, const uint32_t* sorted, const uint32_t* starts, const uint32_t* counts,
                     const uint32_t* order, uint32_t total, void* out_proj, hipStream_t st);
};
const MsmOps* msm_ops_mnt4753_g1();
const MsmOps* msm_ops_mnt4753_g2();
const MsmOps* msm_ops_mnt6753_g1();
const MsmOps* msm_ops_mnt6753_g2();
const MsmOps* ops_of(gh_curve_t curve);

int fft_run(gh_field_t field, void* d_data, uint32_t log_n, uint32_t flags);
int vec_op(gh_field_t field, int op, void* d_a, const void* d_b, const uint64_t* scalar12, size_t n);
int witness_map(gh_field_t field, void* d_a, void* d_b, void* d_c, uint32_t log_n, const uint64_t* d1,
                const uint64_t* d2, const uint64_t* d3, void* d_h);
int sap_witness_map(gh_field_t field, void* d_a, void* d_c, uint32_t log_n, const uint64_t* d1, const uint64_t* d2, void* d_h);
int batch_inverse(gh_field_t field, void* d_a, size_t n);
int lagrange_coefficients(gh_field_t field, uint32_t log_n, const uint64_t* tau12, void* d_out);
int domain_table(gh_field_t field, uint32_t log_n, const gh::Fp** tw);

struct FixedTable;
int fixed_table_create(gh_curve_t curve, const uint64_t* g_xyz, size_t scalar_size, int window, FixedTable** out);
int fixed_table_sums(const FixedTable* t, const void* d_scalars, size_t n, void* d_out_proj);
void fixed_table_destroy(FixedTable* t);
int poseidon_field(const gh_poseidon* h, gh_field_t* out);
int poseidon_hash_dev_locked(gh_poseidon* h, const void* d_in, size_t n, size_t len, void* d_out);
void poseidon_trim_slab();
int points_member_dev(gh_curve_t curve, const void* d_xy, const uint8_t* d_inf, size_t n, uint8_t* d_code, size_t stride);
int points_decompress_dev(gh_curve_t curve, const void* d_x, const uint8_t* d_flags, size_t n, void* d_xy, uint8_t* d_inf, uint8_t* d_code, size_t stride);
int points_validate_mark(int end);
int points_validate_finish();

}
```

ginger-lib_amd/gm17.py:

```python
import contextlib
import time

import numpy as np

from . import sap
from .limbs import FR_FIELD, MODULUS, affine_to_wire, canon_rows, domain_size, ints_from_canon_rows, ints_from_mont_rows, mont_rows
from .prover import ResidentQueries, into_repr, upload_rows


def sap_rows_from_r1cs(pairing, num_inputs, assignment, A, B, C):
    r = MODULUS[pairing]
    n_con = len(A)
    ni = num_inputs
    full = list(assignment)
    n_var = len(full)
    extra = [(x - y) * (x - y) % r for x, y in zip(A, B)]
    full += extra
    for i in range(1, ni):
        full.append((full[i] - 1) * (full[i] - 1) % r)
    size = domain_size(2 * n_con + 2 * (ni - 1) + 1)
    off = 2 * n_con
    var_off, var_off2 = n_var, n_var + n_con - 1
    a = [0] * size
    c = [0] * size
    for i in range(n_con):
        a[2 * i] = (A[i] + B[i]) % r
        a[2 * i + 1] = (A[i] - B[i]) % r
        c[2 * i] = (4 * C[i] + full[var_off + i]) % r
        c[2 * i + 1] = full[var_off + i]
    a[off] = 1
    c[off] = 1
    for i in range(1, ni):
        a[off + 2 * i - 1] = (full[i] + 1) % r
        a[off + 2 * i] = (full[i] - 1) % r
        c[off + 2 * i - 1] = (4 * full[i] + full[var_off2 + i]) % r
        c[off + 2 * i] = full[var_off2 + i]
    return full, a, c, size.bit_length() - 1


class ResidentGm17Key(ResidentQueries):

    def __init__(self, gl, pairing, pk, num_inputs, precompute=True):
        super().__init__(gl, pairing, num_inputs)
        row = lambda v: np.asarray(v, dtype=np.uint64).reshape(1, -1)
        cat = lambda *parts: np.ascontiguousarray(np.concatenate(parts), dtype=np.uint64)
        def flags(q, head_last, tail):
            f = pk.get(q + "_inf")
            if f is None:
                return None
            f = np.asarray(f, dtype=np.uint8)
            f = np.concatenate([f[1:], f[:1]]) if head_last else f
            return np.ascontiguousarray(np.concatenate([f, np.zeros(tail, dtype=np.uint8)]))
        self._upload({
            "a": (self.g1, cat(pk["a_query"][1:], row(pk["a_query"][0]), row(pk["g_gamma_z"])), flags("a_query", True, 1)),
            "b": (self.g2, cat(pk["b_query"][1:], row(pk["b_query"][0]), row(pk["h_gamma_z"])), flags("b_query", True, 1)),
            "c1": (self.g1, cat(pk["c_query_1"], row(pk["g_gamma2_z2"]), row(pk["g_ab_gamma_z"])), flags("c_query_1", False, 2)),
            "c2": (self.g1, cat(pk["c_query_2"][1:], row(pk["c_query_2"][0])), flags("c_query_2", True, 0)),
            "g": (self.g1, cat(pk["g_gamma2_z_t"], row(pk["g_gamma2_z_t"][0])), None),
        }, precompute)

    def create_proof_msms(self, input_assignment, aux_assignment, h, d1, d2, r, h_dev=None, scalars_dev=None):
        gl, ni = self.gl, self.num_inputs
        g1, g2 = self.g1, self.g2
        mod = MODULUS[self.pairing]
        k = self.keys
        n_var = k["a"].n - 2
        assert k["b"].n - 2 == n_var and k["c2"].n - 1 == n_var and k["c1"].n - 2 == n_var - (ni - 1)
        n_aux = n_var - (ni - 1)
        s_tail = [canon_rows([1]), canon_rows([(r + d1) % mod])]
        c1_tail = [canon_rows([(r * r + 2 * r * d1) % mod, (r + d1) % mod])]
        row_d2 = canon_rows([d2 % mod])
        with contextlib.ExitStack() as stack:
            if scalars_dev is not None:
                d_s, d_c1, n = scalars_dev[0], scalars_dev[1], int(scalars_dev[2])
                if n != n_var or d_s.nbytes < (n + 2) * 96 or d_c1.nbytes < (n_aux + 2) * 96:
                    raise ValueError("the scalar vectors must hold one row per variable of the key's queries, and room for two more each")
                upload_rows(gl, d_s, s_tail, n_var)
                upload_rows(gl, d_c1, c1_tail, n_aux)
            else:
                inp = np.ascontiguousarray(input_assignment, dtype=np.uint64).reshape(-1, 12)
                aux = np.ascontiguousarray(aux_assignment, dtype=np.uint64).reshape(-1, 12)
                assert len(inp) == ni - 1
                aux_used = aux[:n_aux]
                pad = np.zeros((n_aux - len(aux_used), 12), dtype=np.uint64)
                d_s = stack.enter_context(gl.DeviceBuffer((n_var + 2) * 96))
                d_c1 = stack.enter_context(gl.DeviceBuffer((n_aux + 2) * 96))
                assert upload_rows(gl, d_s, [inp, aux_used, pad] + s_tail) == n_var + 2
                assert upload_rows(gl, d_c1, [aux_used, pad] + c1_tail) == n_aux + 2
            if h_dev is None:
                h_all = np.ascontiguousarray(h, dtype=np.uint64).reshape(-1, 12)
                n_h = min(len(h_all), k["g"].n - 1)
                hv = np.concatenate([h_all[:n_h], np.zeros((k["g"].n - 1 - n_h, 12), dtype=np.uint64), row_d2])
                d_h = stack.enter_context(gl.DeviceBuffer(hv.nbytes)).upload(hv)
            else:
                d_h, n_h = h_dev[0], int(h_dev[1])
                assert n_h == k["g"].n - 1
                upload_rows(gl, d_h, [row_d2], n_h)
            g_a, c1, c2, g_acc = gl.msm_batch_dev([(k["a"], d_s, n_var + 2), (k["c1"], d_c1, n_var - (ni - 1) + 2),
                                                   (k["c2"], d_s, n_var + 1), (k["g"], d_h, k["g"].n)])
            g_b = k["b"].msm_dev(d_s, n_var + 2)
        g_c = gl.proj_add(g1, c1, gl.proj_mul(g1, c2, canon_rows([r % mod])[0]))
        g_c = gl.proj_add(g1, g_c, g_acc)
        return gl.proj_to_affine(g1, g_a), gl.proj_to_affine(g2, g_b), gl.proj_to_affine(g1, g_c)

    def prepare_rows(self, circuit_rows, d1, d2):
        mod = MODULUS[self.pairing]
        num_inputs, assignment, A, B, C = circuit_rows
        assert num_inputs == self.num_inputs
        full, a, c, log_n = sap_rows_from_r1cs(self.pairing, num_inputs, assignment, A, B, C)
        return {"size": 1 << log_n, "a": mont_rows(a, mod), "c": mont_rows(c, mod), "dd": mont_rows([d1, d2], mod), "scal": canon_rows(full),
                "d1": d1, "d2": d2}

    def prove_prepared(self, prep, r, timing=None):
        gl, num_inputs = self.gl, self.num_inputs
        size, dd, scal = prep["size"], prep["dd"], prep["scal"]
        log_n = size.bit_length() - 1
        field = FR_FIELD[self.pairing]
        lib = gl.load_library()
        t0 = time.perf_counter()
        with contextlib.ExitStack() as stack:
            bufs = [stack.enter_context(gl.DeviceBuffer(size * 96 + 192)) for _ in range(3)]
            bufs[0].upload(prep["a"])
            bufs[1].upload(prep["c"])
            lib.gh_dev_sync()
            t1 = time.perf_counter()
            gl._check(lib.gh_sap_witness_map_dev(gl.FIELDS[field], bufs[0].ptr, bufs[1].ptr, log_n, gl._ptr(dd[0]), gl._ptr(dd[1]), bufs[2].ptr))
            into_repr(gl, field, bufs[2], size + 1)
            lib.gh_dev_sync()
            t2 = time.perf_counter()
            n_h = self.keys["g"].n - 1
            assert n_h <= size + 1
            proof = self.create_proof_msms(scal[1:num_inputs], scal[num_inputs:], None, prep["d1"], prep["d2"], r, h_dev=(bufs[2], n_h))
            t3 = time.perf_counter()
        if timing is not None:
            timing.update(rows_upload_ms=(t1 - t0) * 1e3, witness_map_ms=(t2 - t1) * 1e3, msm_stage_ms=(t3 - t2) * 1e3)
        return proof

    def create_proof(self, circuit_rows, d1, d2, r):
        return self.prove_prepared(self.prepare_rows(circuit_rows, d1, d2), r)

    def create_proof_r1cs(self, r1cs, assignment, d1, d2, r, timing=None):
        gl = self.gl
        mod = MODULUS[self.pairing]
        if r1cs.num_inputs != self.num_inputs:
            raise ValueError("the constraint system and the key disagree on the number of inputs")
        z = assignment if isinstance(assignment, np.ndarray) else mont_rows(list(assignment), mod)
        z = np.ascontiguousarray(z, dtype=np.uint64).reshape(-1, 12)
        nv = r1cs.num_variables
        if len(z) != nv:
            raise ValueError("the assignment must have one row per variable")
        info = sap.sap_info(r1cs)
        size, sap_nv = info["size"], info["sap_num_variables"]
        n_aux = sap_nv - (self.num_inputs - 1)
        n_h = self.keys["g"].n - 1
        if n_h > size + 1:
            raise ValueError("the key's g_gamma2_z_t query is longer than h")
        dd = mont_rows([d1, d2], mod)
        lib = gl.load_library()
        t0 = time.perf_counter()
        with contextlib.ExitStack() as stack:
            d_z, d_h, d_s, d_c1 = (stack.enter_context(gl.DeviceBuffer(rows * 96)) for rows in (nv, size + 2, sap_nv + 2, n_aux + 2))
            d_z.upload(z)
            lib.gh_dev_sync()
            t1 = time.perf_counter()
            sap.sap_witness_map_dev(r1cs, d_z, dd, d_h, d_s, d_c1)
            into_repr(gl, FR_FIELD[self.pairing], d_h, size + 1)
            lib.gh_dev_sync()
            t2 = time.perf_counter()
            proof = self.create_proof_msms(None, None, None, d1, d2, r, h_dev=(d_h, n_h), scalars_dev=(d_s, d_c1, sap_nv))
            t3 = time.perf_counter()
        if timing is not None:
            timing.update(assignment_upload_ms=(t1 - t0) * 1e3, witness_map_ms=(t2 - t1) * 1e3, msm_stage_ms=(t3 - t2) * 1e3)
        return proof


def sap_instance_map_host(lcs, u, r):
    num_inputs, num_aux, at, bt, ct = lcs
    n_con = len(at)
    ni1 = num_inputs - 1
    sap_nv = 2 * ni1 + num_aux + n_con
    xvo, xco, xvo2 = ni1 + num_aux + 1, 2 * n_con, ni1 + num_aux + n_con
    a, c = [0] * (sap_nv + 1), [0] * (sap_nv + 1)
    for i in range(n_con):
        u0, u1 = u[2 * i], u[2 * i + 1]
        ua, us = (u0 + u1) % r, (u0 - u1) % r
        for cf, ix in at[i]:
            a[ix] = (a[ix] + ua * cf) % r
        for cf, ix in bt[i]:
            a[ix] = (a[ix] + us * cf) % r
        for cf, ix in ct[i]:
            c[ix] = (c[ix] + 4 * u0 * cf) % r
        c[xvo + i] = (c[xvo + i] + ua) % r
    a[0] = (a[0] + u[xco]) % r
    c[0] = (c[0] + u[xco]) % r
    for i in range(1, ni1 + 1):
        uo, ue = u[xco + 2 * i - 1], u[xco + 2 * i]
        a[i] = (a[i] + uo + ue) % r
        a[0] = (a[0] + uo - ue) % r
        c[i] = (c[i] + 4 * uo) % r
        c[xvo2 + i] = (c[xvo2 + i] + uo + ue) % r
    return a, c


def _instance_map_on_device(gl, field, r1cs, shape, tau):
    num_inputs, num_aux, n_con, log_n = shape
    if (r1cs.num_inputs, r1cs.num_aux, r1cs.num_constraints) != shape[:3] or sap.sap_info(r1cs)["sap_log_n"] != log_n:
        raise ValueError("the resident constraint system is not the one of lcs")
    rows = 2 * (num_inputs - 1) + num_aux + n_con + 1
    with contextlib.ExitStack() as stack:
        d_u = stack.enter_context(gl.DeviceBuffer(96 << log_n))
        outs = [stack.enter_context(gl.DeviceBuffer(rows * 96)) for _ in range(2)]
        gl._check(gl.load_library().gh_lagrange_coefficients_dev(gl.FIELDS[field], log_n, gl._ptr(tau), d_u.ptr))
        sap.sap_instance_map_dev(r1cs, d_u, *outs)
        res = []
        for o in outs:
            into_repr(gl, field, o, rows)
            res.append(ints_from_canon_rows(o.download()[:rows * 12]))
        return tuple(res)


def generate_parameters(gl, pairing, lcs, alpha, beta, gamma, t, g1_xyz, g2_xyz, r1cs=None):
    r = MODULUS[pairing]
    field = FR_FIELD[pairing]
    g1c, g2c = pairing + "_g1", pairing + "_g2"
    num_inputs, num_aux, at, bt, ct = lcs
    n_con = len(at)
    ni1 = num_inputs - 1
    size = domain_size(2 * n_con + 2 * ni1 + 1)
    log_n = size.bit_length() - 1
    zt = (pow(t, size, r) - 1) % r
    tau = mont_rows([t], r)[0]
    sap_nv = 2 * ni1 + num_aux + n_con
    if r1cs is not None:
        a, c = _instance_map_on_device(gl, field, r1cs, (num_inputs, num_aux, n_con, log_n), tau)
    else:
        u_rows = np.zeros((size, 12), dtype=np.uint64)
        gl._check(gl.load_library().gh_lagrange_coefficients(gl.FIELDS[field], log_n, gl._ptr(tau), gl._ptr(u_rows)))
        a, c = sap_instance_map_host(lcs, ints_from_mont_rows(u_rows, r), r)
    non_zero_a = sum(1 for v in a[:sap_nv] if v)
    m_raw = size
    FB = gl.FixedBaseMSM
    g_window = FB.get_mul_window_size(num_inputs + non_zero_a + (sap_nv - ni1) + sap_nv + 1 + m_raw + 1)
    h_window = FB.get_mul_window_size(non_zero_a)
    ab = (alpha + beta) % r
    gz = gamma * zt % r
    stats = {"fixed_base_scalars": 0, "fixed_base_calls": 0}

    def rows(table, vals):
        xy, inf = table.multi_scalar_mul_affine(canon_rows(vals), canonical=False)
        stats["fixed_base_scalars"] += len(vals)
        stats["fixed_base_calls"] += 1
        return np.ascontiguousarray(xy, dtype=np.uint64), np.asarray(inf, dtype=np.uint8)

# ... 58 lines not shown
```

ginger-lib_amd/groth16.py:

```python
import contextlib
import struct
import time

import numpy as np

from .limbs import FQ_BYTES, FQK_BYTES, FR_FIELD, G2_DEG, MODULUS, affine_to_wire, canon_rows, domain_size, ints_from_canon_rows, \
    ints_from_mont_rows, mont_rows
from .prover import ResidentQueries, RowView, into_repr, upload_rows


def parse_parameters(pairing, blob):
    g1 = 2 * FQ_BYTES + 1
    g2 = 2 * FQ_BYTES * G2_DEG[pairing] + 1
    pos = 0

    def take(nbytes):
        nonlocal pos
        if pos + nbytes > len(blob):
            raise ValueError("Parameters stream is truncated")
        out = bytes(blob[pos:pos + nbytes])
        pos += nbytes
        return out

    def vec(rec):
# ... 145 lines not shown
        a[i] = u[n_con + i]
    for rows, acc in ((at, a), (bt, b), (ct, c)):
        for i, row in enumerate(rows):
            ui = u[i]
            for cf, ix in row:
                acc[ix] = (acc[ix] + (ui if cf == 1 else ui * cf)) % r
    return a, b, c


def _instance_map_on_device(gl, field, r1cs, shape, tau):
    num_inputs, num_aux, n_con, log_n = shape
    if (r1cs.num_inputs, r1cs.num_aux, r1cs.num_constraints, r1cs.log_n) != shape:
        raise ValueError("the resident constraint system is not the one of lcs")
    nv1 = num_inputs + num_aux
    with contextlib.ExitStack() as stack:
        d_u = stack.enter_context(gl.DeviceBuffer(96 << log_n))
        outs = [stack.enter_context(gl.DeviceBuffer(nv1 * 96)) for _ in range(3)]
        gl._check(gl.load_library().gh_lagrange_coefficients_dev(gl.FIELDS[field], log_n, gl._ptr(tau), d_u.ptr))
        r1cs.instance_map_dev(d_u, *outs)
        res = []
        for o in outs:
            into_repr(gl, field, o, nv1)
            res.append(ints_from_canon_rows(o.download()[:nv1 * 12]))
        return tuple(res)


class ResidentProvingKey(ResidentQueries):

    def __init__(self, gl, pairing, pk, num_inputs, precompute=True):
        super().__init__(gl, pairing, num_inputs)
        row = lambda v: np.asarray(v, dtype=np.uint64).reshape(1, -1)
        def ext(q, c, d, delta_last):
            dl = row(pk[d])
            tail = [np.zeros_like(dl), dl] if delta_last else [dl, np.zeros_like(dl)]
            rows = np.ascontiguousarray(np.concatenate([pk[q][1:], row(pk[q][0]), row(pk[c])] + tail), dtype=np.uint64)
            inf = np.zeros(len(rows), dtype=np.uint8)
            inf[-2 if delta_last else -1] = 1
            return rows, inf
        self._init_queries({"a": (self.g1,) + ext("a_query", "alpha_g1", "delta_g1", False),
                            "b1": (self.g1,) + ext("b_g1_query", "beta_g1", "delta_g1", True),
                            "b2": (self.g2,) + ext("b_g2_query", "beta_g2", "delta_g2", True),
                            "h": (self.g1, np.ascontiguousarray(pk["h_query"], dtype=np.uint64), None),
                            "l": (self.g1, np.ascontiguousarray(pk["l_query"], dtype=np.uint64), None)}, pk["delta_g1"], precompute)

    @classmethod
    def from_parameters(cls, gl, pairing, blob, num_inputs, precompute=True):
        self = cls.__new__(cls)
        ResidentQueries.__init__(self, gl, pairing, num_inputs)
        pk = parse_parameters(pairing, blob)
        r1, r2 = 2 * FQ_BYTES + 1, 2 * FQ_BYTES * G2_DEG[pairing] + 1
        def ext(q, c, d, rec, delta_last):
            zero = bytes(rec - 1) + b"\x01"
            tail = zero + pk[d] if delta_last else pk[d] + zero
            return pk[q][rec:] + pk[q][:rec] + pk[c] + tail
        self._init_queries({"a": (self.g1, ext("a_query", "alpha_g1", "delta_g1", r1, False)),
                            "b1": (self.g1, ext("b_g1_query", "beta_g1", "delta_g1", r1, True)),
                            "b2": (self.g2, ext("b_g2_query", "beta_g2", "delta_g2", r2, True)),
                            "h": (self.g1, pk["h_query"]), "l": (self.g1, pk["l_query"])}, pk["delta_g1"], precompute)
        return self

    def _init_queries(self, vectors, delta_g1, precompute):
        if isinstance(delta_g1, bytes):
            one = self.gl.ResidentBases.from_wire(self.g1, delta_g1)
            try:
                delta_g1 = one.download(0, 1)[0]
            finally:
                one.free()
        self.delta_g1 = np.asarray(delta_g1, dtype=np.uint64).ravel()
        self._upload(vectors, precompute)

    def prepare_rows(self, circuit_rows, d1, d2, d3):
        modulus = MODULUS[self.pairing]
        num_inputs, assignment, A, B, C = circuit_rows
        assert num_inputs == self.num_inputs
        n_con = len(A)
        size = domain_size(n_con + num_inputs)
        a = np.zeros((size, 12), dtype=np.uint64)
        b = np.zeros((size, 12), dtype=np.uint64)
        c = np.zeros((size, 12), dtype=np.uint64)
        a[:n_con] = mont_rows(A, modulus)
        b[:n_con] = mont_rows(B, modulus)
        c[:n_con] = mont_rows(C, modulus)
        a[n_con:n_con + num_inputs] = mont_rows([1] + list(assignment[1:num_inputs]), modulus)
        return {"size": size, "a": a, "b": b, "c": c, "dd": mont_rows([d1, d2, d3], modulus), "scal": canon_rows(assignment)}

    def prove_prepared(self, prep, r, s, timing=None):
        gl = self.gl
        size, num_inputs = prep["size"], self.num_inputs
        log_n = size.bit_length() - 1
        field = FR_FIELD[self.pairing]
        dd, scal = prep["dd"], prep["scal"]
        lib = gl.load_library()
        t0 = time.perf_counter()
        with contextlib.ExitStack() as stack:
            bufs = [stack.enter_context(gl.DeviceBuffer(size * 96 + 96)) for _ in range(4)]
            for buf, arr in zip(bufs, (prep["a"], prep["b"], prep["c"])):
                buf.upload(arr)
            lib.gh_dev_sync()
            t1 = time.perf_counter()
            gl._check(lib.gh_witness_map_dev(gl.FIELDS[field], bufs[0].ptr, bufs[1].ptr, bufs[2].ptr, log_n, gl._ptr(dd[0]), gl._ptr(dd[1]),
                                             gl._ptr(dd[2]), bufs[3].ptr))
            into_repr(gl, field, bufs[3], size + 1)
            lib.gh_dev_sync()
            t2 = time.perf_counter()
            proof = self.create_proof_msms(scal[1:num_inputs], scal[num_inputs:], None, None, canon_rows([r])[0], canon_rows([s])[0],
                                           h_dev=(bufs[3], self.keys["h"].n))
            t3 = time.perf_counter()
        if timing is not None:
            timing.update(rows_upload_ms=(t1 - t0) * 1e3, witness_map_ms=(t2 - t1) * 1e3, msm_stage_ms=(t3 - t2) * 1e3)
        return self._proof_bytes(proof)

    def _proof_bytes(self, proof):
        return b"".join(affine_to_wire(self.pairing, group, *pt) for group, pt in zip(("g1", "g2", "g1"), proof))

    def create_proof(self, circuit_rows, d1, d2, d3, r, s):
        return self.prove_prepared(self.prepare_rows(circuit_rows, d1, d2, d3), r, s)

    def create_proof_msms(self, input_assignment, aux_assignment, h_input_assignment, h_aux_assignment, r, s, h_dev=None, scalars_dev=None):
        gl, ni, k = self.gl, self.num_inputs, self.keys
        n_var = k["a"].n - 4
        if k["b1"].n - 4 != n_var or k["b2"].n - 4 != n_var:
            raise ValueError("the a, b_g1 and b_g2 queries of the key differ in length")
        r = np.ascontiguousarray(r, dtype=np.uint64).reshape(1, 12)
        s = np.ascontiguousarray(s, dtype=np.uint64).reshape(1, 12)
        one = canon_rows([1])
        tail = np.concatenate([one, one, r, s])
        if scalars_dev is not None:
            d_s, n = scalars_dev[0], int(scalars_dev[1])
            if n != n_var or d_s.nbytes < (n + 4) * 96:
                raise ValueError("the scalar vector must hold one row per variable of the key's queries, and room for four more")
            upload_rows(gl, d_s, [tail], n)
            return self._msm_stage(d_s, r, s, h_dev[0], int(h_dev[1]), RowView(d_s, ni - 1), n - (ni - 1))
        inp = np.ascontiguousarray(input_assignment, dtype=np.uint64).reshape(-1, 12)
        aux = np.ascontiguousarray(aux_assignment, dtype=np.uint64).reshape(-1, 12)
        assert len(inp) == ni - 1 and n_var >= len(inp)
        aux_used = aux[:n_var - len(inp)]
        pad = np.zeros((n_var - len(inp) - len(aux_used), 12), dtype=np.uint64)
        with contextlib.ExitStack() as stack:
            alloc = lambda nbytes: stack.enter_context(gl.DeviceBuffer(nbytes))
            d_s = alloc((n_var + 4) * 96)
            assert upload_rows(gl, d_s, (inp, aux_used, pad, tail)) == n_var + 4
            if h_dev is not None:
                d_h, n_h = h_dev[0], int(h_dev[1])
            else:
                h_all = np.concatenate([np.ascontiguousarray(h_input_assignment, dtype=np.uint64).reshape(-1, 12),
                                        np.ascontiguousarray(h_aux_assignment, dtype=np.uint64).reshape(-1, 12)])
                d_h, n_h = alloc(max(96, h_all.nbytes)).upload(h_all), len(h_all)
            d_l = RowView(d_s, ni - 1) if len(aux_used) == len(aux) else alloc(max(96, aux.nbytes)).upload(aux)
            return self._msm_stage(d_s, r, s, d_h, n_h, d_l, len(aux))

    def _msm_stage(self, d_s, r, s, d_h, n_h, d_l, n_l):
        gl, g1, g2, k = self.gl, self.g1, self.g2, self.keys
        add, mul = gl.proj_add, gl.proj_mul
        g_a, g1_b, h_acc, l_acc = gl.msm_batch_dev([(k["a"], d_s, k["a"].n), (k["b1"], d_s, k["a"].n), (k["h"], d_h, n_h), (k["l"], d_l, n_l)])
        g2_b = k["b2"].msm_dev(d_s, k["a"].n)
        delta = np.concatenate([self.delta_g1, gl.field_one(g1)])
        g_c = add(g1, mul(g1, g_a, s), mul(g1, g1_b, r))
        g_c = add(g1, g_c, gl.proj_neg(g1, mul(g1, mul(g1, delta, r), s)))
        g_c = add(g1, g_c, l_acc)
        g_c = add(g1, g_c, h_acc)
        return gl.proj_to_affine(g1, g_a), gl.proj_to_affine(g2, g2_b), gl.proj_to_affine(g1, g_c)

    def create_proof_r1cs(self, r1cs, assignment, d1, d2, d3, r, s, timing=None):
        gl = self.gl
        modulus = MODULUS[self.pairing]
        if r1cs.num_inputs != self.num_inputs:
            raise ValueError("the constraint system and the key disagree on the number of inputs")
        z = assignment if isinstance(assignment, np.ndarray) else mont_rows(list(assignment), modulus)
        z = np.ascontiguousarray(z, dtype=np.uint64).reshape(-1, 12)
        nv, size = r1cs.num_variables, r1cs.size
        if len(z) != nv:
            raise ValueError("the assignment must have one row per variable")
        dd = mont_rows([d1, d2, d3], modulus)
        lib = gl.load_library()
        t0 = time.perf_counter()
        with contextlib.ExitStack() as stack:
            d_z, d_h, d_s = (stack.enter_context(gl.DeviceBuffer(nbytes)) for nbytes in (nv * 96, size * 96 + 96, (nv + 3) * 96))
            d_z.upload(z)
            lib.gh_dev_sync()
            t1 = time.perf_counter()
            r1cs.witness_map_dev(d_z, dd, d_h, d_s)
            into_repr(gl, FR_FIELD[self.pairing], d_h, size + 1)
            lib.gh_dev_sync()
            t2 = time.perf_counter()
            proof = self.create_proof_msms(None, None, None, None, canon_rows([r])[0], canon_rows([s])[0],
                                           h_dev=(d_h, self.keys["h"].n), scalars_dev=(d_s, nv - 1))
            t3 = time.perf_counter()
        if timing is not None:
            timing.update(assignment_upload_ms=(t1 - t0) * 1e3, witness_map_ms=(t2 - t1) * 1e3, msm_stage_ms=(t3 - t2) * 1e3)
        return self._proof_bytes(proof)
```

rust/algebra-hip-sys/src/lib.rs:

```rust
#![allow(non_camel_case_types)]

use std::ffi::CStr;
use std::os::raw::{c_char, c_int, c_void};

#[repr(C)]
pub struct GhBases {
    _private: [u8; 0],
}

#[repr(C)]
pub struct GhFixedTable {
    _private: [u8; 0],
}

#[repr(C)]
#[derive(Clone, Copy, Debug, Default)]
pub struct GhMsmTiming {
    pub sort_ms: f32,
    pub accumulate_ms: f32,
    pub heavy_ms: f32,
    pub reduce_ms: f32,
    pub fold_ms: f32,
    pub total_ms: f32,
    pub window_bits: c_int,
// ... 107 lines not shown
    pub fn gh_dist_probe_rccl() -> c_int;
    pub fn gh_dist_info(rank: *mut c_int, world: *mut c_int) -> c_int;
    pub fn gh_dist_transport(rccl_ranks: *mut c_int, rccl_version: *mut c_int, path: *mut c_char, path_cap: usize) -> c_int;
    pub fn gh_partials_allgather_fold(curve: c_int, partial_xyz: *const u64, out_xyz: *mut u64, exchange_us: *mut f64) -> c_int;
    pub fn gh_partials_allgather_fold_batch(curve: c_int, partials_xyz: *const u64, count: usize, outs_xyz: *mut u64, exchange_us: *mut f64) -> c_int;
    pub fn gh_dist_shutdown() -> c_int;
}

pub fn curve_degree(curve: c_int) -> usize {
    match curve {
        MNT4753_G2 => 2,
        MNT6753_G2 => 3,
        _ => 1,
    }
}

pub fn last_error() -> String {
    unsafe {
        let p = gh_last_error();
        if p.is_null() {
            String::new()
        } else {
            CStr::from_ptr(p).to_string_lossy().into_owned()
        }
    }
}

fn status(rc: c_int) -> Result<(), c_int> {
    if rc == GH_OK {
        Ok(())
    } else {
        Err(rc)
    }
}

pub fn msm(curve: c_int, bases: &[u64], infinity: &[u8], scalars: &[u64]) -> Result<Vec<u64>, c_int> {
    let deg = curve_degree(curve);
    if bases.len() != infinity.len() * 24 * deg || scalars.len() % 12 != 0 {
        return Err(GH_E_BAD_ARG);
    }
    let mut out = vec![0u64; 36 * deg];
    status(unsafe {
        gh_msm(curve, bases.as_ptr(), infinity.as_ptr(), infinity.len(), scalars.as_ptr(), scalars.len() / 12, out.as_mut_ptr())
    })?;
    Ok(out)
}

pub struct ResidentBases {
    handle: *mut GhBases,
    curve: c_int,
    len: usize,
}

unsafe impl Send for ResidentBases {}
unsafe impl Sync for ResidentBases {}

impl ResidentBases {
    pub fn upload(curve: c_int, bases: &[u64], infinity: &[u8]) -> Result<Self, c_int> {
        let deg = curve_degree(curve);
        if bases.len() != infinity.len() * 24 * deg {
            return Err(GH_E_BAD_ARG);
        }
        let mut handle: *mut GhBases = std::ptr::null_mut();
        status(unsafe { gh_bases_upload(curve, bases.as_ptr(), infinity.as_ptr(), infinity.len(), &mut handle) })?;
        Ok(ResidentBases { handle, curve, len: infinity.len() })
    }

    pub fn upload_wire(curve: c_int, bytes: &[u8]) -> Result<Self, c_int> {
        let rec = 192 * curve_degree(curve) + 1;
        if bytes.len() % rec != 0 {
            return Err(GH_E_BAD_ARG);
        }
        let mut handle: *mut GhBases = std::ptr::null_mut();
        status(unsafe { gh_bases_upload_wire(curve, bytes.as_ptr(), bytes.len() / rec, &mut handle) })?;
        Ok(ResidentBases { handle, curve, len: bytes.len() / rec })
    }

    pub fn precompute(&self, window_bits: c_int) -> Result<c_int, c_int> {
        status(unsafe { gh_bases_precompute(self.handle, window_bits) })?;
        Ok(unsafe { gh_bases_precomputed_window(self.handle) })
    }

    pub fn precompute_rows(&self, window_bits: c_int, max_rows: c_int) -> Result<c_int, c_int> {
        status(unsafe { gh_bases_precompute_rows(self.handle, window_bits, max_rows) })?;
        Ok(unsafe { gh_bases_table_rows(self.handle) })
    }

    pub fn len(&self) -> usize {
        self.len
    }

    pub fn is_empty(&self) -> bool {
        self.len == 0
    }

    pub fn curve(&self) -> c_int {
        self.curve
    }

    pub fn raw(&self) -> *mut GhBases {
        self.handle
    }

    pub fn msm(&self, scalars: &[u64]) -> Result<Vec<u64>, c_int> {
        if scalars.len() % 12 != 0 {
            return Err(GH_E_BAD_ARG);
        }
        let mut out = vec![0u64; 36 * curve_degree(self.curve)];
        status(unsafe { gh_msm_resident(self.handle, scalars.as_ptr(), scalars.len() / 12, out.as_mut_ptr()) })?;
        Ok(out)
    }
}

impl Drop for ResidentBases {
    fn drop(&mut self) {
        unsafe {
            gh_bases_free(self.handle);
        }
    }
}

pub fn msm_cached(curve: c_int, bases: &[u64], infinity: &[u8], scalars: &[u64]) -> Result<Vec<u64>, c_int> {
    let deg = curve_degree(curve);
    if bases.len() != infinity.len() * 24 * deg || scalars.len() % 12 != 0 {
        return Err(GH_E_BAD_ARG);
    }
    let mut out = vec![0u64; 36 * deg];
    status(unsafe {
        gh_msm_cached(curve, bases.as_ptr(), infinity.as_ptr(), infinity.len(), scalars.as_ptr(), scalars.len() / 12, out.as_mut_ptr())
    })?;
    Ok(out)
}

pub fn key_cache_config(max_bytes: usize, table_after: c_int) -> Result<(), c_int> {
    status(unsafe { gh_key_cache_config(max_bytes, table_after) })
}

pub fn key_cache_stats() -> Result<GhKeyCacheStats, c_int> {
    let mut st = GhKeyCacheStats::default();
    status(unsafe { gh_key_cache_stats(&mut st) })?;
    Ok(st)
}

pub fn clear_keys() {
    unsafe {
        gh_key_cache_clear();
    }
}

pub fn msm_batch(jobs: &[(&ResidentBases, &[u64])]) -> Result<Vec<Vec<u64>>, c_int> {
    if jobs.is_empty() {
        return Ok(Vec::new());
    }
    let curve = jobs[0].0.curve;
    let deg = curve_degree(curve);
    let mut dev: Vec<*mut c_void> = Vec::with_capacity(jobs.len());
    let mut result = Err(GH_E_BAD_ARG);
    'run: loop {
        for (key, scalars) in jobs {
            if key.curve != curve || scalars.len() % 12 != 0 {
                break 'run;
            }
            let mut p: *mut c_void = std::ptr::null_mut();
            let bytes = std::cmp::max(96, scalars.len() * 8);
            let rc = unsafe { gh_dev_alloc(&mut p, bytes) };
            if rc != GH_OK {
                result = Err(rc);
                break 'run;
            }
            dev.push(p);
            let rc = unsafe { gh_dev_upload(p, scalars.as_ptr() as *const c_void, scalars.len() * 8) };
            if rc != GH_OK {
                result = Err(rc);
                break 'run;
            }
        }
        let handles: Vec<*mut GhBases> = jobs.iter().map(|j| j.0.handle).collect();
        let ptrs: Vec<*const c_void> = dev.iter().map(|p| *p as *const c_void).collect();
        let lens: Vec<usize> = jobs.iter().map(|j| j.1.len() / 12).collect();
        let mut out = vec![0u64; jobs.len() * 36 * deg];
        let rc = unsafe {
            gh_msm_resident_dev_batch(handles.as_ptr(), ptrs.as_ptr(), lens.as_ptr(), jobs.len() as c_int, out.as_mut_ptr())
        };
        result = if rc == GH_OK { Ok(out.chunks(36 * deg).map(|c| c.to_vec()).collect()) } else { Err(rc) };
        break;
    }
    for p in dev {
        unsafe {
            gh_dev_free(p);
        }
    }
    result
}

pub fn domain_log_size(field: c_int, num_coeffs: usize) -> Option<u32> {
    let mut lg = 0u32;
    if unsafe { gh_domain_supported(field, num_coeffs, &mut lg) } == 1 {
        Some(lg)
    } else {
        None
    }
}

pub fn fft(field: c_int, data: &[u64], log_n: u32, flags: u32) -> Result<Vec<u64>, c_int> {
    if data.len() % 12 != 0 || log_n >= 31 {
        return Err(GH_E_BAD_ARG);
    }
    let mut out = vec![0u64; 12usize << log_n];
    status(unsafe { gh_fft(field, data.as_ptr(), data.len() / 12, out.as_mut_ptr(), log_n, flags) })?;
    Ok(out)
}

pub fn vec_mul(field: c_int, a: &mut [u64], b: &[u64]) -> Result<(), c_int> {
    if a.len() != b.len() || a.len() % 12 != 0 {
        return Err(GH_E_BAD_ARG);
    }
    status(unsafe { gh_vec_mul(field, a.as_mut_ptr(), b.as_ptr(), a.len() / 12) })
}

pub fn vec_scale(field: c_int, a: &mut [u64], s: &[u64; 12]) -> Result<(), c_int> {
    if a.len() % 12 != 0 {
        return Err(GH_E_BAD_ARG);
    }
    status(unsafe { gh_vec_scale(field, a.as_mut_ptr(), s.as_ptr(), a.len() / 12) })
}

pub fn witness_map(field: c_int, a: &[u64], b: &[u64], c: &[u64], log_n: u32, d1: &[u64; 12], d2: &[u64; 12], d3: &[u64; 12]) -> Result<Vec<u64>, c_int> {
    let n = 12usize << log_n;
    if a.len() != n || b.len() != n || c.len() != n {
        return Err(GH_E_BAD_ARG);
    }
    let mut h = vec![0u64; n + 12];
    status(unsafe { gh_witness_map(field, a.as_ptr(), b.as_ptr(), c.as_ptr(), log_n, d1.as_ptr(), d2.as_ptr(), d3.as_ptr(), h.as_mut_ptr()) })?;
    Ok(h)
}

pub struct FixedBaseTable {
    handle: *mut GhFixedTable,
    curve: c_int,
}
unsafe impl Send for FixedBaseTable {}
unsafe impl Sync for FixedBaseTable {}

impl FixedBaseTable {
    pub fn window_size(num_scalars: usize) -> usize {
        unsafe { gh_fixed_base_window(num_scalars) as usize }
    }
    pub fn new(curve: c_int, g_xyz: &[u64], scalar_size: usize, window: usize) -> Result<Self, c_int> {
        if g_xyz.len() != 36 * curve_degree(curve) {
            return Err(GH_E_BAD_ARG);
        }
        let mut handle: *mut GhFixedTable = std::ptr::null_mut();
        status(unsafe { gh_fixed_base_table(curve, g_xyz.as_ptr(), scalar_size, window as c_int, &mut handle) })?;
        Ok(FixedBaseTable { handle, curve })
    }
    pub fn multi_scalar_mul(&self, scalars: &[u64]) -> Result<Vec<u64>, c_int> {
        if scalars.len() % 12 != 0 {
            return Err(GH_E_BAD_ARG);
        }
        let n = scalars.len() / 12;
        let mut out = vec![0u64; n * 36 * curve_degree(self.curve)];
        status(unsafe { gh_fixed_base_msm(self.handle, scalars.as_ptr(), n, out.as_mut_ptr()) })?;
        Ok(out)
    }
}
impl Drop for FixedBaseTable {
    fn drop(&mut self) {
        unsafe {
            gh_fixed_base_free(self.handle);
        }
    }
}

pub fn proj_add(curve: c_int, acc: &mut [u64], p: &[u64]) -> Result<(), c_int> {
    let w = 36 * curve_degree(curve);
    if acc.len() != w || p.len() != w {
        return Err(GH_E_BAD_ARG);
    }
    status(unsafe { gh_proj_add(curve, acc.as_mut_ptr(), p.as_ptr()) })
}

pub fn partials_allgather_fold(curve: c_int, partial: &[u64]) -> Result<Vec<u64>, c_int> {
    let w = 36 * curve_degree(curve);
    if partial.len() != w {
        return Err(GH_E_BAD_ARG);
    }
    let mut out = vec![0u64; w];
    status(unsafe { gh_partials_allgather_fold(curve, partial.as_ptr(), out.as_mut_ptr(), std::ptr::null_mut()) })?;
    Ok(out)
}

pub mod poseidon;

pub mod schnorr;

pub mod ecvrf;

pub mod pairing;

pub mod gm17;

pub mod points;

pub mod r1cs;

pub mod sap;
```

Measured before the change: 56.18 million.

## Allow mixed-curve MSM batches with a unified job pipeline and pre-reserved buffers

Replaces the per-curve batch and run functions with a polymorphic MsmJobBase driven by a single scheduler that overlaps the sort, accumulate and reduce stages across jobs on several streams. Batches may now mix one G1 curve and one extension-field G2 curve, so the Groth16 and GM17 provers fold the G2 B MSM into the same batch instead of running it afterwards. Buffer needs are computed up front and reserved once before any job is issued. The aim is to overlap the G2 MSM with the G1 jobs and avoid allocations in the middle of the pipeline, at the cost of more complex stream and event coordination.

```diff
diff --git a/ginger-lib_amd/__init__.py b/ginger-lib_amd/__init__.py
--- a/ginger-lib_amd/__init__.py
+++ b/ginger-lib_amd/__init__.py
@@ -335,17 +335,24 @@
             self.handle = ctypes.c_void_p()
 
 
+def batch_result_offsets(curves):
+    offsets = [0]
+    for curve in curves:
+        offsets.append(offsets[-1] + 36 * CURVE_DEG[curve])
+    return offsets
+
+
 def msm_batch_dev(jobs):
     if not jobs:
         return []
     k = len(jobs)
-    deg = CURVE_DEG[jobs[0][0].curve]
+    off = batch_result_offsets([j[0].curve for j in jobs])
     handles = (ctypes.c_void_p * k)(*[j[0].handle for j in jobs])
     scal = (ctypes.c_void_p * k)(*[j[1].ptr for j in jobs])
     ns = (ctypes.c_size_t * k)(*[int(j[2]) for j in jobs])
-    out = np.zeros(k * 36 * deg, dtype=np.uint64)
+    out = np.zeros(off[-1], dtype=np.uint64)
     _check(load_library().gh_msm_resident_dev_batch(handles, scal, ns, k, _ptr(out)))
-    return [out[i * 36 * deg:(i + 1) * 36 * deg].copy() for i in range(k)]
+    return [out[off[i]:off[i + 1]].copy() for i in range(k)]
 
 
 class VariableBaseMSM:
diff --git a/ginger-lib_amd/csrc/ginger_hip.hip b/ginger-lib_amd/csrc/ginger_hip.hip
--- a/ginger-lib_amd/csrc/ginger_hip.hip
+++ b/ginger-lib_amd/csrc/ginger_hip.hip
@@ -1,6 +1,7 @@
 #include <atomic>
 #include <condition_variable>
 #include <exception>
+#include <memory>
 #include <new>
 #include <random>
 #include <thread>
@@ -166,13 +167,17 @@
     }
 }
 
+static size_t scan_blocks(size_t n) {
+    const size_t per_block = (size_t)gh::SCAN_BLOCK * gh::SCAN_ITEMS;
+    return (n + per_block - 1) / per_block;
+}
+size_t device_scan_tmp_bytes(size_t n) { return (scan_blocks(n) + 1) * 4; }
 int device_scan(const uint32_t* in, uint32_t* out, size_t n, const char* tmpname, hipStream_t stream) {
     using namespace gh;
     if (!stream) stream = g.stream;
-    size_t per_block = (size_t)SCAN_BLOCK * SCAN_ITEMS;
-    size_t nblocks = (n + per_block - 1) / per_block;
+    const size_t nblocks = scan_blocks(n);
     uint32_t* sums;
-    int rc = pool_get(tmpname, (nblocks + 1) * 4, (void**)&sums);
+    int rc = pool_get(tmpname, device_scan_tmp_bytes(n), (void**)&sums);
     if (rc) return rc;
     GH_LAUNCH(scan_partials_kernel, dim3((unsigned)nblocks), dim3(SCAN_BLOCK), 0, stream, in, sums, n);
     GH_LAUNCH(scan_block_sums_kernel, dim3(1), dim3(1024), 0, stream, sums, nblocks);
@@ -189,6 +194,80 @@
         case GH_MNT6753_G2: return msm_ops_mnt6753_g2();
         default: g_err = "unknown curve id"; return nullptr;
     }
+}
+
+int msm_pinned(int set, int which, size_t bytes, void** out) {
+    static void* p[4][2] = {};
+    static size_t cap[4][2] = {};
+    static bool registered = false;
+    if (!registered) {
+        registered = true;
+        g.at_shutdown.push_back([] {
+            for (auto& sl : p) for (auto& q : sl) { if (q) hipHostFree(q); q = nullptr; }
+            for (auto& sl : cap) for (auto& q : sl) q = 0;
+            registered = false;
+        });
+    }
+    if (cap[set][which] < bytes) {
+        if (p[set][which]) HIPCHK(hipHostFree(p[set][which]));
+        p[set][which] = nullptr; cap[set][which] = 0;
+        HIPCHK(hipHostMalloc(&p[set][which], bytes + 256, hipHostMallocDefault));
+        cap[set][which] = bytes + 256;
+    }
+    *out = p[set][which];
+    return GH_OK;
+}
+
+static int msm_batch_issue(BasesBase* const* hs, const void* const* d_scalars, const size_t* n_scalars, int count, uint64_t* out_xyz,
+                           std::vector<std::unique_ptr<MsmJobBase>>& jobs) {
+    int rc;
+    BufNeeds needs;
+    size_t out_off = 0;
+    for (int k = 0; k < count; k++) {
+        const MsmOps* ops = ops_of(hs[k]->curve);
+        if (!ops) return GH_E_BAD_ARG;
+        jobs[(size_t)k].reset(ops->make_job());
+        MsmJobBase& j = *jobs[(size_t)k];
+        j.solo = count == 1;
+        j.last = k == count - 1;
+        j.es = k & 3;
+        j.slot = k & 1;
+        if ((rc = j.plan(hs[k], d_scalars[k], n_scalars[k], out_xyz + out_off)) || (rc = j.buffers(needs))) return rc;
+        out_off += j.out_stride();
+    }
+    if ((rc = needs.reserve())) return rc;
+    auto issue_sort = [&](int k) -> int {
+        MsmJobBase& j = *jobs[(size_t)k];
+        if ((rc = j.prepare())) return rc;
+        if (k >= 2) {
+            HIPCHK(hipStreamWaitEvent(g.stream, g.pev[(k - 2) & 3][4], 0));
+        }
+        return j.launch_sort(g.stream);
+    };
+    if ((rc = issue_sort(0))) return rc;
+    for (int k = 0; k < count; k++) {
+        MsmJobBase& j = *jobs[(size_t)k];
+        const bool sort_first = j.tree && j.n && k + 1 < count;
+        if (sort_first && (rc = issue_sort(k + 1))) return rc;
+        const bool alt = j.is_g1() && g.stream_acc_alt && gh_asm::enabled() && msm_knobs().acc_persist && (k & 1);
+        const hipStream_t st_acc = alt ? g.stream_acc_alt : g.stream_acc;
+        if (k >= 2 && j.n) HIPCHK(hipStreamWaitEvent(st_acc, g.pev[(k - 2) & 3][6], 0));
+        if ((rc = j.launch_accumulate(st_acc))) return rc;
+        if (j.n) HIPCHK(hipStreamWaitEvent(g.stream_red, g.pev[k & 3][4], 0));
+        if ((rc = j.launch_reduce(g.stream_red))) return rc;
+        if (!sort_first && k + 1 < count && (rc = issue_sort(k + 1))) return rc;
+        if (k >= 1 && (rc = jobs[(size_t)k - 1]->finish())) return rc;
+    }
+    return jobs[(size_t)count - 1]->finish();
+}
+
+int msm_batch_jobs(BasesBase* const* hs, const void* const* d_scalars, const size_t* n_scalars, int count, uint64_t* out_xyz) {
+    g.batch_tm.clear();
+    if (count <= 0) return GH_OK;
+    std::vector<std::unique_ptr<MsmJobBase>> jobs((size_t)count);
+    const int rc = msm_batch_issue(hs, d_scalars, n_scalars, count, out_xyz, jobs);
+    if (rc) (void)sync_msm_streams();
+    return rc;
 }
 
 static int to_device(void* d_dst, const void* h_src, size_t bytes) {
@@ -355,11 +434,10 @@
     BasesBase* h = bases_of(handle);
     if (!h) { g_err = "bad bases handle"; return GH_E_BAD_HANDLE; }
     if (!out_xyz || (n_scalars && !d_scalars)) { g_err = "null argument"; return GH_E_BAD_ARG; }
-    const MsmOps* ops = ops_of(h->curve);
-    if (!ops) return GH_E_BAD_ARG;
-    int rc = ensure_init();
-    if (rc) return rc;
-    return ops->run(h, d_scalars, n_scalars, out_xyz);
+    if (!ops_of(h->curve)) return GH_E_BAD_ARG;
+    int rc = ensure_init();
+    if (rc) return rc;
+    return msm_run(h, d_scalars, n_scalars, out_xyz);
 } catch (...) { return gh_rt::api_exception(); }
 
 int gh_msm_resident_dev_batch(const gh_bases_t* handles, const void* const* d_scalars, const size_t* n_scalars, int count,
@@ -368,22 +446,20 @@
     if (count < 0 || (count > 0 && (!handles || !d_scalars || !n_scalars || !out_xyz))) { g_err = "null argument"; return GH_E_BAD_ARG; }
     if (count == 0) return GH_OK;
     std::vector<BasesBase*> hs((size_t)count);
+    const BasesBase* of_group[2] = {nullptr, nullptr};
     for (int i = 0; i < count; i++) {
         BasesBase* h = bases_of(handles[i]);
         if (!h) { g_err = "bad bases handle"; return GH_E_BAD_HANDLE; }
         hs[(size_t)i] = h;
-        if (h->curve != hs[0]->curve) { g_err = "a batch must stay on one curve"; return GH_E_BAD_ARG; }
+        if (!ops_of(h->curve)) return GH_E_BAD_ARG;
+        const BasesBase*& first = of_group[curve_deg(h->curve) > 1];
+        if (!first) first = h;
+        if (h->curve != first->curve) { g_err = "a batch must stay on one curve"; return GH_E_BAD_ARG; }
         if (n_scalars[i] && !d_scalars[i]) { g_err = "null argument"; return GH_E_BAD_ARG; }
     }
-    const MsmOps* ops = ops_of(hs[0]->curve);
-    if (!ops) return GH_E_BAD_ARG;
-    int rc = ensure_init();
-    if (rc) return rc;
-    rc = ops->batch(hs.data(), d_scalars, n_scalars, count, out_xyz);
-    if (rc) {
-        (void)sync_msm_streams();
-    }
-    return rc;
+    int rc = ensure_init();
+    if (rc) return rc;
+    return msm_batch_jobs(hs.data(), d_scalars, n_scalars, count, out_xyz);
 } catch (...) { return gh_rt::api_exception(); }
 
 int gh_msm_resident(gh_bases_t handle, const uint64_t* scalars, size_t n_scalars, uint64_t* out_xyz) try {
@@ -391,8 +467,7 @@
     BasesBase* h = bases_of(handle);
     if (!h) { g_err = "bad bases handle"; return GH_E_BAD_HANDLE; }
     if (!out_xyz || (n_scalars && !scalars)) { g_err = "null argument"; return GH_E_BAD_ARG; }
-    const MsmOps* ops = ops_of(h->curve);
-    if (!ops) return GH_E_BAD_ARG;
+    if (!ops_of(h->curve)) return GH_E_BAD_ARG;
     int rc = ensure_init();
     if (rc) return rc;
     const size_t n = h->n < n_scalars ? h->n : n_scalars;
@@ -402,7 +477,7 @@
         if (rc) return rc;
         HIPCHK(hipMemcpyAsync(d_s, scalars, n * 96, hipMemcpyHostToDevice, g.stream));
     }
-    return ops->run(h, d_s, n, out_xyz);
+    return msm_run(h, d_s, n, out_xyz);
 } catch (...) { return gh_rt::api_exception(); }
 
 namespace {
@@ -697,7 +772,7 @@
     cache_fit(key);
     if (uploader.joinable()) uploader.join();
     HIPCHK(up_err);
-    return ops->run(key, d_s, n, out_xyz);
+    return msm_run(key, d_s, n, out_xyz);
 } catch (...) { return gh_rt::api_exception(); }
 
 int gh_msm_set_window(int c) try {
diff --git a/ginger-lib_amd/csrc/msm_impl.h b/ginger-lib_amd/csrc/msm_impl.h
--- a/ginger-lib_amd/csrc/msm_impl.h
+++ b/ginger-lib_amd/csrc/msm_impl.h
@@ -164,24 +164,21 @@
 };
 
 template <class C>
-struct MsmJob {
+struct MsmJob final : MsmJobBase {
     typedef typename SplitFS<C>::type FS;
     static constexpr int DEG = C::F::DEG;
 
     BasesBase* h = nullptr;
     const void* d_scalars = nullptr;
     uint64_t* out_xyz = nullptr;
-    size_t n = 0;
-    int slot = 0;
-    bool solo = false;
-    bool last = false;
-    int es = 0;
     MsmPlan p;
-    bool tree = false;
+    SortPlan sp;
     uint32_t n_heavy = 0, n_chunks = 0;
     int32_t* digits = nullptr;
     uint32_t *counts = nullptr, *starts = nullptr, *cursor = nullptr, *sorted = nullptr, *order = nullptr, *size_hist = nullptr,
-             *size_cursor = nullptr, *chunk_start = nullptr, *plan = nullptr;
+             *size_cursor = nullptr, *chunk_start = nullptr, *plan_words = nullptr;
+    uint32_t *merged_s = nullptr, *merged_partial = nullptr, *block_hist = nullptr, *block_off = nullptr, *slabs = nullptr;
+    uint2* part = nullptr;
     Proj<C>*buckets = nullptr, *seg_out = nullptr, *win_out = nullptr, *partials = nullptr, *lane_out = nullptr;
     uint32_t* red_flag = nullptr;
     uint32_t *aff_cnt = nullptr, *aff_st = nullptr;
@@ -192,32 +189,12 @@
     std::chrono::steady_clock::time_point t_begin;
     gh_msm_timing_t tm{};
 
-    static int pinned(int slot, int which, size_t bytes, void** out) {
-        static void* p[4][2] = {};
-        static size_t cap[4][2] = {};
-        static bool registered = false;
-        if (!registered) {
-            registered = true;
-            g.at_shutdown.push_back([] {
-                for (auto& sl : p) for (auto& q : sl) { if (q) hipHostFree(q); q = nullptr; }
-                for (auto& sl : cap) for (auto& q : sl) q = 0;
-                registered = false;
-            });
-        }
-        if (cap[slot][which] < bytes) {
-            if (p[slot][which]) HIPCHK(hipHostFree(p[slot][which]));
-            p[slot][which] = nullptr; cap[slot][which] = 0;
-            HIPCHK(hipHostMalloc(&p[slot][which], bytes + 256, hipHostMallocDefault));
-            cap[slot][which] = bytes + 256;
-        }
-        *out = p[slot][which];
-        return GH_OK;
-    }
-
-    int prepare(BasesBase* h_, const void* d_scalars_, size_t n_scalars, uint64_t* out, int slot_) {
-        h = h_; d_scalars = d_scalars_; out_xyz = out; slot = slot_;
+    bool is_g1() const override { return DEG == 1; }
+    size_t out_stride() const override { return (size_t)36 * DEG; }
+
+    int plan(BasesBase* h_, const void* d_scalars_, size_t n_scalars, uint64_t* out) override {
+        h = h_; d_scalars = d_scalars_; out_xyz = out;
         n = h->n < n_scalars ? h->n : n_scalars;
-        t_begin = std::chrono::steady_clock::now();
         if (n == 0) return GH_OK;
         p = plan_msm(n, DEG, h->d_table != nullptr, h->pre_c, h->pre_G, solo, last, g.window_override, g.affine_mode, msm_knobs());
         if (p.status == MSM_PLAN_TOO_LARGE) {
@@ -225,35 +202,59 @@
             return GH_E_UNSUPPORTED;
         }
         tree = p.tree;
-        if (int src = device_salts<C>(&salts)) return src;
-        int rc;
-        if ((rc = slot_buf("digits", slot, p.entries * 4, &digits)) ||
-            (rc = slot_buf("counts", slot, p.total * 4, &counts)) ||
-            (rc = slot_buf("starts", slot, p.total * 4, &starts)) ||
-            (rc = slot_buf("cursor", slot, p.total * 4, &cursor)) ||
-            (rc = slot_buf("sorted", slot, p.entries * 4, &sorted)) ||
-            (rc = slot_buf("order", slot, p.total * 4, &order)) ||
-            (rc = slot_buf("size_hist", slot, MSM_SIZE_BINS * 4, &size_hist)) ||
-            (rc = slot_buf("size_cursor", slot, MSM_SIZE_BINS * 4, &size_cursor)) ||
-            (rc = slot_buf("chunk_start", slot, (p.max_heavy + 2) * 4, &chunk_start)) ||
-            (rc = slot_buf("plan", slot, 64, &plan)) ||
-            (rc = slot_buf("buckets", slot, p.total * sizeof(Proj<C>), &buckets)) ||
-            (rc = slot_buf("seg_out", slot, (size_t)p.RW * p.segs_per_window * 3 * sizeof(Proj<C>), &seg_out)) ||
-            (rc = slot_buf("win_out", slot, (size_t)3 * p.RW * 3 * sizeof(Proj<C>), &win_out)))
+        sp = plan_sort(p.entries, n, p.total, msm_knobs());
+        return device_salts<C>(&salts);
+    }
+
+    int buffers(BufVisitor& v) override {
+        if (n == 0) return GH_OK;
+        int rc;
+        auto sb = [&](const char* name, size_t bytes, auto** out) { return v.dev(slot_name(name, slot), bytes, (void**)out); };
+        if ((rc = sb("digits", p.entries * 4, &digits)) ||
+            (rc = sb("counts", p.total * 4, &counts)) ||
+            (rc = sb("starts", p.total * 4, &starts)) ||
+            (rc = sb("cursor", p.total * 4, &cursor)) ||
+            (rc = sb("sorted", p.entries * 4, &sorted)) ||
+            (rc = sb("order", p.total * 4, &order)) ||
+            (rc = sb("size_hist", MSM_SIZE_BINS * 4, &size_hist)) ||
+            (rc = sb("size_cursor", MSM_SIZE_BINS * 4, &size_cursor)) ||
+            (rc = sb("chunk_start", (p.max_heavy + 2) * 4, &chunk_start)) ||
+            (rc = sb("plan", 64, &plan_words)) ||
+            (rc = sb("buckets", p.total * sizeof(Proj<C>), &buckets)) ||
+            (rc = sb("seg_out", (size_t)p.RW * p.segs_per_window * 3 * sizeof(Proj<C>), &seg_out)) ||
+            (rc = sb("win_out", (size_t)3 * p.RW * 3 * sizeof(Proj<C>), &win_out)))
             return rc;
-        if (p.lane_buf && (rc = slot_buf("lane_out", slot, (size_t)p.RW * p.segs_per_window * 64 * 2 * sizeof(Proj<C>), &lane_out))) return rc;
-        if (p.lane_buf && (rc = slot_buf("reduce_flag", slot, (size_t)p.RW * p.segs_per_window * 4 + 64, &red_flag))) return rc;
-        if ((rc = pinned(es, 0, 512, (void**)&hplan))) return rc;
-        if ((rc = pinned(es, 1, (size_t)9 * p.RW * sizeof(Proj<C>), (void**)&hw))) return rc;
-        return GH_OK;
+        if (p.lane_buf && (rc = sb("lane_out", (size_t)p.RW * p.segs_per_window * 64 * 2 * sizeof(Proj<C>), &lane_out))) return rc;
+        if (p.lane_buf && (rc = sb("reduce_flag", (size_t)p.RW * p.segs_per_window * 4 + 64, &red_flag))) return rc;
+        const size_t nb1 = (size_t)p.RW * p.segs_per_window, nb2 = (size_t)3 * p.RW;
+        size_t slab_words;
+        if constexpr (DEG >= 2) slab_words = WaveSlab<P3>::WORDS; else slab_words = WaveSlab<Proj<C>>::WORDS;
+        if ((rc = sb("reduce_slabs", (nb1 > nb2 ? nb1 : nb2) * slab_words * 4, &slabs))) return rc;
+        if (h->n_dup_groups && ((rc = sb("merged_scalars", n * 96, &merged_s)) ||
+                                (rc = sb("merged_partial", (size_t)h->n_dup_chunks * 96 + 96, &merged_partial)))) return rc;
+        void* scan_tmp;
+        if (sp.part) {
+            const size_t cells = (size_t)sp.n_bins * sp.n_blocks + 1;
+            if ((rc = sb("part_hist", cells * 4, &block_hist)) ||
+                (rc = sb("part_off", cells * 4, &block_off)) ||
+                (rc = sb("part_pairs", p.entries * 8, &part)) ||
+                (rc = sb("scan_tmp3", device_scan_tmp_bytes(cells), &scan_tmp))) return rc;
+        } else if ((rc = v.dev("scan_tmp", device_scan_tmp_bytes(p.total), &scan_tmp))) return rc;
+        if ((rc = v.dev("scan_tmp2", device_scan_tmp_bytes(MSM_SIZE_BINS), &scan_tmp))) return rc;
+        if (tree && (rc = sb("aff_scan", device_scan_tmp_bytes(p.total), &scan_tmp))) return rc;
+        if ((rc = v.pin(es, 0, 512, (void**)&hplan))) return rc;
+        return v.pin(es, 1, (size_t)9 * p.RW * sizeof(Proj<C>), (void**)&hw);
+    }
+
+    int prepare() override {
+        t_begin = std::chrono::steady_clock::now();
+        BufAcquire acquire;
+        return buffers(acquire);
     }
 
     int merge_equal_bases(hipStream_t st) {
-        int rc;
-        uint32_t *merged_s = nullptr, *partial = nullptr;
-        if ((rc = slot_buf("merged_scalars", slot, n * 96, &merged_s))) return rc;
+        uint32_t* const partial = merged_partial;
         HIPCHK(hipMemcpyAsync(merged_s, d_scalars, n * 96, hipMemcpyDeviceToDevice, st));
-        if ((rc = slot_buf("merged_partial", slot, (size_t)h->n_dup_chunks * 96 + 96, &partial))) return rc;
         GH_LAUNCH(msm_merge_scalars_kernel, dim3(h->n_dup_chunks), dim3(256), 0, st, (const uint32_t*)d_scalars, merged_s, n,
                   (const uint32_t*)h->d_dup_starts, (const uint32_t*)h->d_dup_members, (const uint32_t*)h->d_dup_chunks, h->n_dup_chunks,
                   partial, scalar_modulus<C>());
@@ -270,7 +271,7 @@
         return GH_OK;
     }
 
-    int sort_partitioned(const SortPlan& sp, hipStream_t st) {
+    int sort_partitioned(hipStream_t st) {
         int rc;
         MsmPartArgs a;
         a.digits = digits; a.entries = p.entries; a.n = n;
@@ -279,11 +280,6 @@
         a.bin_shift = sp.bin_shift; a.n_bins = sp.n_bins;
         a.tile = sp.tile; a.n_blocks = sp.n_blocks;
         const size_t cells = (size_t)a.n_bins * a.n_blocks + 1;
-        uint32_t *block_hist = nullptr, *block_off = nullptr;
-        uint2* part = nullptr;
-        if ((rc = slot_buf("part_hist", slot, cells * 4, &block_hist)) ||
-            (rc = slot_buf("part_off", slot, cells * 4, &block_off)) ||
-            (rc = slot_buf("part_pairs", slot, p.entries * 8, &part))) return rc;
         if ((rc = launch_digits(nullptr, st))) return rc;
         HIPCHK(hipMemsetAsync(block_hist + (cells - 1), 0, 4, st));
         GH_LAUNCH(msm_part_hist_kernel, dim3(a.n_blocks), dim3(MSM_PART_THREADS), 0, st, a, block_hist);
@@ -296,17 +292,16 @@
         return GH_OK;
     }
 
-    int launch_sort(hipStream_t st) {
+    int launch_sort(hipStream_t st) override {
         if (n == 0) return GH_OK;
         int rc;
         const size_t total = p.total;
         HIPCHK(hipEventRecord(g.pev[es][0], st));
         HIPCHK(hipMemsetAsync(size_hist, 0, MSM_SIZE_BINS * 4, st));
-        HIPCHK(hipMemsetAsync(plan, 0, 64, st));
+        HIPCHK(hipMemsetAsync(plan_words, 0, 64, st));
         if (h->n_dup_groups && (rc = merge_equal_bases(st))) return rc;
-        const SortPlan sp = plan_sort(p.entries, n, total, msm_knobs());
         if (sp.part) {
-            if ((rc = sort_partitioned(sp, st))) return rc;
+            if ((rc = sort_partitioned(st))) return rc;
         } else {
             HIPCHK(hipMemsetAsync(counts, 0, total * 4, st));
             if ((rc = launch_digits(counts, st))) return rc;
@@ -314,22 +309,22 @@
             if ((rc = device_scan(counts, starts, total, "scan_tmp", st))) return rc;
             HIPCHK(hipMemcpyAsync(cursor, starts, total * 4, hipMemcpyDeviceToDevice, st));
         }
-        GH_LAUNCH(msm_size_hist_kernel, dim3((unsigned)((total + 255) / 256)), dim3(256), 0, st, counts, total, p.heavy_thr, size_hist, plan + 4);
+        GH_LAUNCH(msm_size_hist_kernel, dim3((unsigned)((total + 255) / 256)), dim3(256), 0, st, counts, total, p.heavy_thr, size_hist, plan_words + 4);
         if ((rc = device_scan(size_hist, size_cursor, MSM_SIZE_BINS, "scan_tmp2", st))) return rc;
         GH_LAUNCH(msm_size_scatter_kernel, dim3((unsigned)((total + 255) / 256)), dim3(256), 0, st, counts, total, p.heavy_thr, size_cursor, order);
         GH_LAUNCH(msm_heavy_plan_kernel, dim3(1), dim3(1), 0, st, (const uint32_t*)size_hist, (const uint32_t*)counts,
-                  (const uint32_t*)order, (const uint32_t*)starts, (uint32_t)total, p.heavy_chunk, chunk_start, plan);
+                  (const uint32_t*)order, (const uint32_t*)starts, (uint32_t)total, p.heavy_chunk, chunk_start, plan_words);
         if (!sp.part)
             GH_LAUNCH(msm_scatter_kernel, dim3((unsigned)((n + 255) / 256), (unsigned)p.W), dim3(256), 0, st,
                       (const int32_t*)digits, n, p.W, p.nb, p.merged ? (uint32_t)h->n : 0u, cursor, sorted, msm_knobs().agg_iters,
                       p.merged ? 1u : 0u, (uint32_t)p.sets);
         HIPCHK(hipGetLastError());
-        HIPCHK(hipMemcpyAsync(hplan, plan, 32, hipMemcpyDeviceToHost, st));
+        HIPCHK(hipMemcpyAsync(hplan, plan_words, 32, hipMemcpyDeviceToHost, st));
         HIPCHK(hipEventRecord(g.pev[es][1], st));
         return GH_OK;
     }
 
-    int launch_accumulate(hipStream_t st) {
+    int launch_accumulate(hipStream_t st) override {
         if (n == 0) return GH_OK;
         int rc;
         HIPCHK(hipEventSynchronize(g.pev[es][1]));
@@ -590,16 +585,12 @@
         return reduce_level(nb1, i0, none, none, nb1, 1u, segs, p.L1, lane_out, slabs, one_wave, st);
     }
 
-    int launch_reduce(hipStream_t st) {
+    int launch_reduce(hipStream_t st) override {
         if (n == 0) return GH_OK;
         int rc;
         const uint32_t RW = (uint32_t)p.RW, segs = p.segs_per_window, all = 0xFFFFFFFFu;
         const unsigned nb1 = RW * segs, nb2 = 3 * RW;
         const WaveReduceIn<C> none{nullptr, 0, 0, 0, 0, 0};
-        uint32_t* slabs = nullptr;
-        size_t slab_words;
-        if constexpr (DEG >= 2) slab_words = WaveSlab<P3>::WORDS; else slab_words = WaveSlab<Proj<C>>::WORDS;
-        if ((rc = slot_buf("reduce_slabs", slot, (size_t)(nb1 > nb2 ? nb1 : nb2) * slab_words * 4, &slabs))) return rc;
         const int env_w = msm_knobs().reduce_waves;
         const bool one_wave = env_w ? env_w == 1 : solo;
         if (p.lean) {
@@ -621,7 +612,7 @@
         return GH_OK;
     }
 
-    int finish() {
+    int finish() override {
         if (n == 0) {
             proj_to_abi_host<C>(out_xyz, proj_zero<C>());
             g.last_msm = gh_msm_timing_t{};
@@ -666,43 +657,7 @@
     return GH_OK;
 }
 
-template <class C>
-int msm_batch(BasesBase* const* hs, const void* const* d_scalars, const size_t* n_scalars, int count, uint64_t* out_xyz) {
-    const size_t out_stride = (size_t)36 * C::F::DEG;
-    std::vector<MsmJob<C>> jobs((size_t)count);
-    int rc;
-    auto issue_sort = [&](int k) -> int {
-        MsmJob<C>& j = jobs[(size_t)k];
-        j.solo = count == 1;
-        j.last = k == count - 1;
-        j.es = k & 3;
-        if ((rc = j.prepare(hs[k], d_scalars[k], n_scalars[k], out_xyz + (size_t)k * out_stride, k & 1))) return rc;
-        if (k >= 2) {
-            HIPCHK(hipStreamWaitEvent(g.stream, g.pev[(k - 2) & 3][4], 0));
-        }
-        return j.launch_sort(g.stream);
-    };
-    g.batch_tm.clear();
-    if (count <= 0) return GH_OK;
-    if ((rc = issue_sort(0))) return rc;
-    for (int k = 0; k < count; k++) {
-        MsmJob<C>& j = jobs[(size_t)k];
-        const bool alt = C::F::DEG == 1 && g.stream_acc_alt && gh_asm::enabled() && msm_knobs().acc_persist && (k & 1);
-        const hipStream_t st_acc = alt ? g.stream_acc_alt : g.stream_acc;
-        if (k >= 2 && j.n) HIPCHK(hipStreamWaitEvent(st_acc, g.pev[(k - 2) & 3][6], 0));
-        if ((rc = j.launch_accumulate(st_acc))) return rc;
-        if (j.n) HIPCHK(hipStreamWaitEvent(g.stream_red, g.pev[k & 3][4], 0));
-        if ((rc = j.launch_reduce(g.stream_red))) return rc;
-        if (k + 1 < count && (rc = issue_sort(k + 1))) return rc;
-        if (k >= 1 && (rc = jobs[(size_t)k - 1].finish())) return rc;
-    }
-    return jobs[(size_t)count - 1].finish();
-}
-
-template <class C>
-int msm_run(BasesBase* h, const void* d_scalars, size_t n_scalars, uint64_t* out_xyz) {
-    return msm_batch<C>(&h, &d_scalars, &n_scalars, 1, out_xyz);
-}
+template <class C> MsmJobBase* make_msm_job() { return new MsmJob<C>(); }
 
 template <class C>
 int msm_host(const uint64_t* bases, const uint8_t* infinity, size_t n_bases, const uint64_t* scalars, size_t n_scalars,
@@ -718,16 +673,16 @@
         hipError_t e = hipMemcpyAsync(d_s, scalars, n * 96, hipMemcpyHostToDevice, g.stream);
         if (e != hipSuccess) { g_err = hipGetErrorString(e); return GH_E_HIP; }
     }
-    return msm_run<C>(h.get(), d_s, n, out_xyz);
+    return msm_run(h.get(), d_s, n, out_xyz);
 }
 
 
 #define GH_DEFINE_MSM_OPS(CURVE, NAME)                                                        \
     namespace gh_rt {                                                                          \
     const MsmOps* NAME() {                                                                     \
-        static const MsmOps ops = {&upload_bases<CURVE>, &msm_run<CURVE>, &msm_host<CURVE>,    \
+        static const MsmOps ops = {&upload_bases<CURVE>, &make_msm_job<CURVE>, &msm_host<CURVE>, \
                                    &proj_add_host<CURVE>, &to_affine_host<CURVE>,              \
-                                   &precompute_bases<CURVE>, &msm_batch<CURVE>,                \
+                                   &precompute_bases<CURVE>,                                   \
                                    &proj_mul_host<CURVE>, &proj_neg_host<CURVE>, &accumulate_lists<CURVE>};           \
         return &ops;                                                                           \
     }                                                                                          \
diff --git a/ginger-lib_amd/csrc/runtime.h b/ginger-lib_amd/csrc/runtime.h
--- a/ginger-lib_amd/csrc/runtime.h
+++ b/ginger-lib_amd/csrc/runtime.h
@@ -88,6 +88,7 @@
     return e;
 }
 int device_scan(const uint32_t* in, uint32_t* out, size_t n, const char* tmpname, hipStream_t stream = nullptr);
+size_t device_scan_tmp_bytes(size_t n);
 inline int auto_window(size_t n, int deg) { return auto_window(n, deg, g.window_override); }
 void dist_teardown_locked();
 
@@ -177,15 +178,68 @@
     BasesBase* h = reinterpret_cast<BasesBase*>(handle);
     return h && h->magic == BasesBase::MAGIC ? h : nullptr;
 }
+struct BufVisitor {
+    virtual ~BufVisitor() = default;
+    virtual int dev(const std::string& pool_name, size_t bytes, void** out) = 0;
+    virtual int pin(int set, int which, size_t bytes, void** out) = 0;
+};
+int msm_pinned(int set, int which, size_t bytes, void** out);
+struct BufAcquire : BufVisitor {
+    int dev(const std::string& pool_name, size_t bytes, void** out) override { return pool_get(pool_name.c_str(), bytes, out); }
+    int pin(int set, int which, size_t bytes, void** out) override { return msm_pinned(set, which, bytes, out); }
+};
+struct BufNeeds : BufVisitor {
+    std::map<std::string, size_t> pool;
+    size_t pinned[4][2] = {};
+    int dev(const std::string& pool_name, size_t bytes, void**) override {
+        size_t& b = pool[pool_name];
+        if (b < bytes) b = bytes;
+        return GH_OK;
+    }
+    int pin(int set, int which, size_t bytes, void**) override {
+        if (pinned[set][which] < bytes) pinned[set][which] = bytes;
+        return GH_OK;
+    }
+    int reserve() const {
+        void* p;
+        for (const auto& kv : pool) if (int rc = pool_get(kv.first.c_str(), kv.second, &p)) return rc;
+        for (int s = 0; s < 4; s++) for (int w = 0; w < 2; w++)
+            if (pinned[s][w]) if (int rc = msm_pinned(s, w, pinned[s][w], &p)) return rc;
+        return GH_OK;
+    }
+};
+
+struct MsmJobBase {
+    size_t n = 0;
+    int slot = 0;
+    int es = 0;
+    bool solo = false;
+    bool last = false;
+    bool tree = false;
+    virtual ~MsmJobBase() = default;
+    virtual bool is_g1() const = 0;
+    virtual size_t out_stride() const = 0;
+    virtual int plan(BasesBase* h, const void* d_scalars, size_t n_scalars, uint64_t* out) = 0;
+    virtual int buffers(BufVisitor& v) = 0;
+    virtual int prepare() = 0;
+    virtual int launch_sort(hipStream_t st) = 0;
+    virtual int launch_accumulate(hipStream_t st) = 0;
+    virtual int launch_reduce(hipStream_t st) = 0;
+    virtual int finish() = 0;
+};
+int msm_batch_jobs(BasesBase* const* hs, const void* const* d_scalars, const size_t* n_scalars, int count, uint64_t* out_xyz);
+inline int msm_run(BasesBase* h, const void* d_scalars, size_t n_scalars, uint64_t* out_xyz) {
+    return msm_batch_jobs(&h, &d_scalars, &n_scalars, 1, out_xyz);
+}
+
 struct MsmOps {
     int (*upload)(const uint64_t* bases, const uint8_t* infinity, size_t n, int canonical, BasesBase** out);
-    int (*run)(BasesBase* h, const void* d_scalars, size_t n_scalars, uint64_t* out_xyz);
+    MsmJobBase* (*make_job)();
     int (*host)(const uint64_t* bases, const uint8_t* infinity, size_t n_bases, const uint64_t* scalars,
                 size_t n_scalars, uint64_t* out_xyz);
     int (*proj_add)(uint64_t* acc_xyz, const uint64_t* p_xyz);
     int (*to_affine)(const uint64_t* xyz, uint64_t* out_xy, uint8_t* is_infinity);
     int (*precompute)(BasesBase* h, int window_bits, int max_rows);
-    int (*batch)(BasesBase* const* hs, const void* const* d_scalars, const size_t* n_scalars, int count, uint64_t* out_xyz);
     int (*proj_mul)(const uint64_t* p_xyz, const uint64_t* scalar12, uint64_t* out_xyz);
     int (*proj_neg)(uint64_t* xyz);
     int (*acc_lists)(const void* points, const uint32_t* sorted, const uint32_t* starts, const uint32_t* counts,
diff --git a/ginger-lib_amd/gm17.py b/ginger-lib_amd/gm17.py
--- a/ginger-lib_amd/gm17.py
+++ b/ginger-lib_amd/gm17.py
@@ -96,9 +96,8 @@
                 d_h, n_h = h_dev[0], int(h_dev[1])
                 assert n_h == k["g"].n - 1
                 upload_rows(gl, d_h, [row_d2], n_h)
-            g_a, c1, c2, g_acc = gl.msm_batch_dev([(k["a"], d_s, n_var + 2), (k["c1"], d_c1, n_var - (ni - 1) + 2),
-                                                   (k["c2"], d_s, n_var + 1), (k["g"], d_h, k["g"].n)])
-            g_b = k["b"].msm_dev(d_s, n_var + 2)
+            g_a, c1, c2, g_acc, g_b = gl.msm_batch_dev([(k["a"], d_s, n_var + 2), (k["c1"], d_c1, n_var - (ni - 1) + 2),
+                                                        (k["c2"], d_s, n_var + 1), (k["g"], d_h, k["g"].n), (k["b"], d_s, n_var + 2)])
         g_c = gl.proj_add(g1, c1, gl.proj_mul(g1, c2, canon_rows([r % mod])[0]))
         g_c = gl.proj_add(g1, g_c, g_acc)
         return gl.proj_to_affine(g1, g_a), gl.proj_to_affine(g2, g_b), gl.proj_to_affine(g1, g_c)
diff --git a/ginger-lib_amd/groth16.py b/ginger-lib_amd/groth16.py
--- a/ginger-lib_amd/groth16.py
+++ b/ginger-lib_amd/groth16.py
@@ -321,8 +321,8 @@
     def _msm_stage(self, d_s, r, s, d_h, n_h, d_l, n_l):
         gl, g1, g2, k = self.gl, self.g1, self.g2, self.keys
         add, mul = gl.proj_add, gl.proj_mul
-        g_a, g1_b, h_acc, l_acc = gl.msm_batch_dev([(k["a"], d_s, k["a"].n), (k["b1"], d_s, k["a"].n), (k["h"], d_h, n_h), (k["l"], d_l, n_l)])
-        g2_b = k["b2"].msm_dev(d_s, k["a"].n)
+        g_a, g1_b, h_acc, l_acc, g2_b = gl.msm_batch_dev([(k["a"], d_s, k["a"].n), (k["b1"], d_s, k["a"].n), (k["h"], d_h, n_h), (k["l"], d_l, n_l),
+                                                          (k["b2"], d_s, k["a"].n)])
         delta = np.concatenate([self.delta_g1, gl.field_one(g1)])
         g_c = add(g1, mul(g1, g_a, s), mul(g1, g1_b, r))
         g_c = add(g1, g_c, gl.proj_neg(g1, mul(g1, mul(g1, delta, r), s)))
diff --git a/rust/algebra-hip-sys/src/lib.rs b/rust/algebra-hip-sys/src/lib.rs
--- a/rust/algebra-hip-sys/src/lib.rs
+++ b/rust/algebra-hip-sys/src/lib.rs
@@ -283,13 +283,12 @@
     if jobs.is_empty() {
         return Ok(Vec::new());
     }
-    let curve = jobs[0].0.curve;
-    let deg = curve_degree(curve);
+    let lens36: Vec<usize> = jobs.iter().map(|j| 36 * curve_degree(j.0.curve)).collect();
     let mut dev: Vec<*mut c_void> = Vec::with_capacity(jobs.len());
     let mut result = Err(GH_E_BAD_ARG);
     'run: loop {
         for (key, scalars) in jobs {
-            if key.curve != curve || scalars.len() % 12 != 0 {
+            if scalars.len() % 12 != 0 {
                 break 'run;
             }
             let mut p: *mut c_void = std::ptr::null_mut();
@@ -309,11 +308,23 @@
         let handles: Vec<*mut GhBases> = jobs.iter().map(|j| j.0.handle).collect();
         let ptrs: Vec<*const c_void> = dev.iter().map(|p| *p as *const c_void).collect();
         let lens: Vec<usize> = jobs.iter().map(|j| j.1.len() / 12).collect();
-        let mut out = vec![0u64; jobs.len() * 36 * deg];
+        let mut out = vec![0u64; lens36.iter().sum()];
         let rc = unsafe {
             gh_msm_resident_dev_batch(handles.as_ptr(), ptrs.as_ptr(), lens.as_ptr(), jobs.len() as c_int, out.as_mut_ptr())
         };
-        result = if rc == GH_OK { Ok(out.chunks(36 * deg).map(|c| c.to_vec()).collect()) } else { Err(rc) };
+        result = if rc == GH_OK {
+            let mut rest: &[u64] = &out;
+            Ok(lens36
+                .iter()
+                .map(|&len| {
+                    let (head, tail) = rest.split_at(len);
+                    rest = tail;
+                    head.to_vec()
+                })
+                .collect())
+        } else {
+            Err(rc)
+        };
         break;
     }
     for p in dev {
```

Result: slower. 55.38 million (-1.4%).
